# williamleif/GraphSAGE

Hardware: NVIDIA H100
Metric: seed_nodes_per_sec (higher is better)
Workload: dtype f32

## Files before the change

graphsage_b200/_lib.py:

```python
import ctypes
import os

import torch

_HERE = os.path.dirname(os.path.abspath(__file__))
LIB_PATH = os.path.join(_HERE, "csrc", "libgraphsage_b200.so")

ABI_VERSION = 2
GS_F32, GS_BF16 = 0, 1
ACT_NONE, ACT_RELU = 0, 1
COMBINE_ADD, COMBINE_CONCAT = 0, 1
MATH_FP32_SIMT, MATH_TF32X3, MATH_TF32, MATH_BF16 = 0, 1, 2, 3
MAX_SEGMENTS = 4

c_i32, c_i64, c_u64, c_vp = ctypes.c_int32, ctypes.c_int64, ctypes.c_uint64, ctypes.c_void_p


class Segment(ctypes.Structure):
    _fields_ = [("self_ids", c_vp), ("neigh_ids", c_vp), ("self_row0", c_i64), ("neigh_row0", c_i64),
                ("n", c_i64), ("k", c_i32), ("_pad", c_i32), ("out_row0", c_i64)]


MAX_SHARDS = 16


class ShardedTable(ctypes.Structure):
    _fields_ = [("base", c_vp * MAX_SHARDS), ("row_start", c_i64 * (MAX_SHARDS + 1)), ("n_shards", c_i32),
                ("my_shard", c_i32), ("n_global_rows", c_i64), ("zero_row", c_i64), ("remap", c_vp)]


class GemmPart(ctypes.Structure):
    _fields_ = [("A", c_vp), ("lda", c_i64), ("K", c_i32), ("B", c_vp), ("ldb", c_i64), ("N", c_i32)]


MAX_EMBED_LISTS = 8
MAX_UNIQUE_SAMPLED = 1024
UNIQUE_DRAW_BUDGET = 1 << 20


class EmbedGradList(ctypes.Structure):
    _fields_ = [("ids", c_vp), ("grad", c_vp), ("ldg", c_i64), ("n", c_i64), ("group", c_i32), ("scale", ctypes.c_float)]


class DropoutSite(ctypes.Structure):
    _fields_ = [("seed", c_u64), ("call", ctypes.c_uint32), ("rate", ctypes.c_float), ("call_dev", c_vp)]


_SIGNATURES = {
    "gs_version": (c_i32, []),
    "gs_last_error_string": (ctypes.c_char_p, []),
    "gs_set_tuning": (c_i32, [ctypes.c_char_p, c_i32]),
    "gs_sample_padded": (c_i32, [c_vp, c_i64, c_i32, c_vp, c_i64, c_i32, c_vp, c_u64, c_u64, c_vp, c_vp, c_vp]),
    "gs_sample_padded_khop": (c_i32, [c_vp, c_i64, c_i32, c_vp, c_i64, ctypes.POINTER(c_i32), c_i32, c_u64, c_u64, c_vp,
                                      ctypes.POINTER(c_vp), c_vp]),
    "gs_build_padded_adj": (c_i32, [c_vp, c_vp, c_i64, c_i32, c_vp, c_u64, c_u64, c_vp, c_vp, c_vp]),
    "gs_sample_unigram": (c_i32, [c_vp, c_i64, c_i32, c_u64, c_u64, c_vp, c_vp, c_vp]),
    "gs_sample_unigram_unique": (c_i32, [c_vp, c_i64, c_i32, c_u64, c_u64, c_vp, c_vp, c_vp, c_vp]),
    "gs_sample_csr": (c_i32, [c_vp, c_vp, c_i64, c_vp, c_i64, c_i32, c_i32, c_u64, c_u64, c_vp, c_i32, c_vp, c_vp]),
    "gs_perm_prefix_host": (c_i32, [c_u64, c_u64, c_i32, c_i32, ctypes.POINTER(c_i32)]),
    "gs_gather_rows": (c_i32, [c_vp, c_i32, c_i64, c_i32, c_i64, c_vp, c_i64, c_vp, c_i64, c_vp]),
    "gs_gather_mean": (c_i32, [c_vp, c_i32, c_i64, c_i32, c_i64, ctypes.POINTER(Segment), c_i32, c_i32, c_vp, c_vp,
                               c_i64, c_vp]),
    "gs_gather_mean_sharded": (c_i32, [ctypes.POINTER(ShardedTable), c_i32, c_i32, c_i64, ctypes.POINTER(Segment), c_i32,
                                       c_i32, c_i32, c_vp, c_vp, c_vp, c_i64, c_vp]),
    "gs_halo_begin": (c_i32, [c_vp, c_i64, c_vp, c_vp]),
    "gs_halo_claim": (c_i32, [ctypes.POINTER(ShardedTable), c_vp, c_i64, c_vp, c_vp, c_vp, c_i64, c_vp]),
    "gs_halo_fetch": (c_i32, [ctypes.POINTER(ShardedTable), c_i32, c_i64, c_vp, c_vp, c_i64, c_vp, c_i64, c_vp]),
    "gs_halo_translate": (c_i32, [ctypes.POINTER(ShardedTable), c_vp, c_i64, c_vp, c_vp, c_vp]),
    "gs_translate_ids": (c_i32, [ctypes.POINTER(ShardedTable), c_vp, c_i64, c_vp, c_vp]),
    "gs_gather_rows_sharded": (c_i32, [ctypes.POINTER(ShardedTable), c_i32, c_i32, c_i64, c_vp, c_i64, c_vp, c_i64, c_vp]),
    "gs_shard_alloc": (c_i32, [c_i64, ctypes.POINTER(c_vp)]),
    "gs_shard_free": (c_i32, [c_vp]),
    "gs_ipc_export": (c_i32, [c_vp, ctypes.c_char_p]),
    "gs_ipc_import": (c_i32, [ctypes.c_char_p, ctypes.POINTER(c_vp)]),
    "gs_ipc_close": (c_i32, [c_vp]),
    "gs_gather_rows_f32": (c_i32, [c_vp, c_i32, c_i64, c_i32, c_i64, c_vp, c_i64, c_i64, c_vp, c_i64, c_vp]),
    "gs_cast_rows_bf16": (c_i32, [c_vp, c_i64, c_i32, c_i64, c_vp, c_i64, c_vp]),
    "gs_rmat_degrees": (c_i32, [c_i32, c_i64, ctypes.c_double, ctypes.c_double, ctypes.c_double, ctypes.c_double,
                                ctypes.c_double, c_u64, c_u64, c_u64, c_u64, c_vp, c_vp]),
    "gs_rmat_fill": (c_i32, [c_i32, c_i64, ctypes.c_double, ctypes.c_double, ctypes.c_double, ctypes.c_double, c_u64, c_u64,
                             c_u64, c_u64, c_vp, c_vp, c_vp, c_i64, c_i64, c_vp]),
    "gs_segment_max": (c_i32, [c_vp, c_i64, c_i32, c_i32, c_i64, c_vp, c_i64, c_vp]),
    "gs_sage_gemm_workspace_bytes": (c_i64, [c_i64, ctypes.POINTER(GemmPart), c_i32, c_i32]),
    "gs_sage_gemm": (c_i32, [c_i64, ctypes.POINTER(GemmPart), c_i32, c_i32, c_vp, c_i32, c_i32, c_vp, c_i64, c_vp,
                             c_vp]),
    "gs_sage_gemm_pack": (c_i32, [ctypes.POINTER(GemmPart), c_i32, c_i32, c_vp, c_vp]),
    "gs_sage_gemm_prepacked": (c_i32, [c_i64, ctypes.POINTER(GemmPart), c_i32, c_i32, c_vp, c_i32, c_i32, c_vp, c_i64,
                                       c_vp, c_vp]),
    "gs_gather_mean_img_bytes": (c_i64, [c_i64, c_i32, c_i32]),
    "gs_gather_mean_img": (c_i32, [c_vp, c_i64, ctypes.POINTER(ShardedTable), c_i32, c_vp, c_i32, c_i64, ctypes.POINTER(Segment),
                                   c_i32, c_i32, c_i32, c_vp, c_vp]),
    "gs_sage_gemm_img": (c_i32, [c_i64, ctypes.POINTER(GemmPart), c_i32, c_i32, c_vp, c_i32, c_vp, c_i64, c_vp, c_vp, c_i32,
                                 c_vp]),
    "gs_sage_layer_small": (c_i32, [c_vp, c_i64, c_i32, c_i64, ctypes.POINTER(Segment), c_i32, ctypes.POINTER(GemmPart),
                                    c_i32, c_i32, c_vp, c_i32, c_i32, c_vp, c_i64, c_vp, c_u64, c_vp]),
    "gs_maxpool_mlp_workspace_bytes": (c_i64, [c_i32, c_i32]),
    "gs_maxpool_mlp_pack": (c_i32, [c_vp, c_i64, c_i32, c_i32, c_vp, c_vp]),
    "gs_maxpool_mlp_fused": (c_i32, [c_vp, c_i64, c_i32, c_i64, c_vp, c_i64, c_i64, c_i32, c_vp, c_vp, c_i32, c_vp, c_i64,
                                     c_vp]),
    "gs_meanpool_mlp_fused": (c_i32, [c_vp, c_i64, c_i32, c_i64, c_vp, c_i64, c_i64, c_i32, c_vp, c_vp, c_i32, c_vp, c_i64,
                                      c_vp]),
    "gs_pipeline_step": (c_i32, [c_vp, c_vp, c_i64, ctypes.POINTER(c_vp), c_i32, c_vp, c_vp, c_i64, c_vp, c_vp, c_vp, c_vp,
                                 c_vp, c_vp]),
    "gs_l2_normalize_rows": (c_i32, [c_vp, c_i64, c_i32, c_i64, c_vp]),
    "gs_bump_counter": (c_i32, [c_vp, c_u64, c_vp]),
    "gs_embedding_grad_workspace_bytes": (c_i64, [ctypes.POINTER(EmbedGradList), c_i32, c_i64, c_i32]),
    "gs_embedding_grad": (c_i32, [ctypes.POINTER(EmbedGradList), c_i32, c_i64, c_i32, c_vp, c_i64, c_vp, c_i64, c_vp]),
    "gs_gather_mean_dropout": (c_i32, [c_vp, c_i64, c_i32, c_i64, ctypes.POINTER(Segment), c_i32, ctypes.POINTER(DropoutSite),
                                       ctypes.POINTER(DropoutSite), c_i32, c_vp, c_vp, c_i64, c_vp]),
    "gs_dropout_apply": (c_i32, [c_vp, c_i64, c_i64, c_i32, c_i32, ctypes.c_float, DropoutSite, c_i32, c_vp, c_i64, c_vp]),
    "gs_embedding_grad_dropout": (c_i32, [ctypes.POINTER(EmbedGradList), ctypes.POINTER(DropoutSite), c_i32, c_i64, c_i32, c_vp,
                                          c_i64, c_vp, c_i64, c_vp]),
    "gs_embedding_sgd": (c_i32, [ctypes.POINTER(EmbedGradList), c_i32, c_i64, c_i32, ctypes.c_float, c_vp, c_i64, c_vp, c_i64,
                                 c_vp]),
    "gs_skipgram_workspace_bytes": (c_i64, [c_i64, c_i32, c_i32]),
    "gs_skipgram_grad": (c_i32, [c_vp, c_i64, c_vp, c_i64, c_i64, c_i32, c_vp, c_vp, c_i64, c_vp, c_i32, c_vp, c_vp, c_vp, c_vp,
                                 c_i64, c_vp, c_vp, c_i64, c_vp, c_i64, c_vp]),
}

_lib = None


def lib():
    global _lib
    if _lib is None:
        if not os.path.exists(LIB_PATH):
            raise ImportError(
                "graphsage_b200: %s is missing - build it with `python -m graphsage_b200.build` "
                "(there is no CPU fallback)" % LIB_PATH)
        _lib = ctypes.CDLL(LIB_PATH)
        for name, (res, args) in _SIGNATURES.items():
            fn = getattr(_lib, name)
            fn.restype, fn.argtypes = res, args
        if _lib.gs_version() != ABI_VERSION:
            raise ImportError("graphsage_b200: %s has ABI version %d, this binding needs %d - rebuild it"
                              % (LIB_PATH, _lib.gs_version(), ABI_VERSION))
        for kv in os.environ.get("GS_TUNING", "").split(","):
            if "=" in kv:
                k, v = kv.split("=", 1)
                _lib.gs_set_tuning(k.strip().encode(), int(v))
    return _lib


def exported_symbols():
    return sorted(_SIGNATURES)


def check(rc):
    if rc != 0:
        msg = lib().gs_last_error_string().decode("utf-8", "replace")
        raise RuntimeError("libgraphsage_b200 error %d: %s" % (rc, msg))


def stream_ptr():
    return torch.cuda.current_stream().cuda_stream


def ptr(t):
    return 0 if t is None else t.data_ptr()


def require_cuda(*tensors):
    for t in tensors:
        if t is not None and not t.is_cuda:
            raise RuntimeError("graphsage_b200: tensor on %s - the hot path is CUDA-only (no CPU fallback)" % t.device)


def set_tuning(key, value):
    return lib().gs_set_tuning(key.encode(), int(value))


def perm_prefix_host(seed, counter, max_deg, k):
    buf = (c_i32 * max(k, 1))()
    check(lib().gs_perm_prefix_host(seed & (2**64 - 1), counter & (2**64 - 1), max_deg, k, buf))
    return list(buf[:k])
```

graphsage_b200/csrc/gather.cu:

```cuda
#include "common.cuh"

namespace gs {

struct SegTable {
  gs_segment s[GS_MAX_SEGMENTS];
  int32_t n_segments;
  int64_t total_rows;
};

__device__ __forceinline__ int find_segment(const SegTable& t, int64_t r, int64_t& local) {
  int si = 0;
  int64_t base = 0, end = 0;
#pragma unroll
  for (int q = 0; q < GS_MAX_SEGMENTS - 1; ++q) {
    if (q < t.n_segments - 1) {
      end += t.s[q].n;
      if (r >= end) {
        base = end;
        si = q + 1;
      }
    }
  }
  local = r - base;
  return si;
}

__device__ __forceinline__ int64_t clamp_row(int64_t id, int64_t n_rows) {
  return (id < 0 || id >= n_rows) ? n_rows - 1 : id;
}

__device__ __forceinline__ float4 mask_tail(float4 v, int col0, int F) {
  if (col0 + 1 >= F) v.y = 0.f;
  if (col0 + 2 >= F) v.z = 0.f;
  if (col0 + 3 >= F) v.w = 0.f;
  return v;
}

template <int kUnroll>
__global__ void __launch_bounds__(256) gather_mean_ldg_kernel(const float* __restrict__ src, int64_t n_src_rows, int F,
                                                              int64_t pitch, const __grid_constant__ SegTable tab, int include_self,
                                                              float* __restrict__ out_self,
                                                              float* __restrict__ out_mean, int64_t out_pitch) {
  const int ncol4 = (int)(out_pitch >> 2);
  for (int64_t r = blockIdx.x; r < tab.total_rows; r += gridDim.x) {
    int64_t i;
    const gs_segment& sg = tab.s[find_segment(tab, r, i)];
    const int k = sg.k;
    const int64_t orow = sg.out_row0 + i;
    const int64_t srow = clamp_row(sg.self_ids ? (int64_t)sg.self_ids[i] : sg.self_row0 + i, n_src_rows);
    for (int c = threadIdx.x; c < ncol4; c += blockDim.x) {
      const int col0 = c * 4;
      float4 acc = make_float4(0.f, 0.f, 0.f, 0.f);
      float4 sv = acc;
      if (col0 < F) {
        int j = 0;
        for (; j + kUnroll <= k; j += kUnroll) {
          float4 v[kUnroll];
#pragma unroll
          for (int u = 0; u < kUnroll; ++u) {
            int64_t nr = clamp_row(sg.neigh_ids ? (int64_t)sg.neigh_ids[i * k + j + u] : sg.neigh_row0 + i * k + j + u,
                                   n_src_rows);
            v[u] = ldg_nc_f4(reinterpret_cast<const float4*>(src + nr * pitch) + c);
          }
#pragma unroll
          for (int u = 0; u < kUnroll; ++u) {
            acc.x += v[u].x; acc.y += v[u].y; acc.z += v[u].z; acc.w += v[u].w;
          }
        }
        for (; j < k; ++j) {
          int64_t nr = clamp_row(sg.neigh_ids ? (int64_t)sg.neigh_ids[i * k + j] : sg.neigh_row0 + i * k + j, n_src_rows);
          float4 v = ldg_nc_f4(reinterpret_cast<const float4*>(src + nr * pitch) + c);
          acc.x += v.x; acc.y += v.y; acc.z += v.z; acc.w += v.w;
        }
        if (include_self || out_self) sv = ldg_nc_f4(reinterpret_cast<const float4*>(src + srow * pitch) + c);
        float div = (float)(k + (include_self ? 1 : 0));
        if (include_self) { acc.x += sv.x; acc.y += sv.y; acc.z += sv.z; acc.w += sv.w; }
        acc.x /= div; acc.y /= div; acc.z /= div; acc.w /= div;
        acc = mask_tail(acc, col0, F);
        sv = mask_tail(sv, col0, F);
      }
      reinterpret_cast<float4*>(out_mean + orow * out_pitch)[c] = acc;
      if (out_self) reinterpret_cast<float4*>(out_self + orow * out_pitch)[c] = sv;
    }
  }
}

struct DropTab {
  DropSite neigh[GS_MAX_SEGMENTS];
  DropSite self[GS_MAX_SEGMENTS];
};

template <bool kDrop>
__global__ void __launch_bounds__(256) gather_mean_scalar_kernel(const float* __restrict__ src, int64_t n_src_rows, int F,
                                                                 int64_t pitch, const __grid_constant__ SegTable tab, int include_self,
                                                                 float* __restrict__ out_self,
                                                                 float* __restrict__ out_mean, int64_t out_pitch,
                                                                 const __grid_constant__ DropTab drop) {
  __shared__ uint32_t drop_off[2 * GS_MAX_SEGMENTS];
  if constexpr (kDrop) {
    if (threadIdx.x < 2 * GS_MAX_SEGMENTS) {
      const int s = threadIdx.x % GS_MAX_SEGMENTS;
      drop_off[threadIdx.x] = drop_call_offset(threadIdx.x < GS_MAX_SEGMENTS ? drop.neigh[s] : drop.self[s]);
    }
    __syncthreads();
  }
  for (int64_t r = blockIdx.x; r < tab.total_rows; r += gridDim.x) {
    int64_t i;
    const int si = find_segment(tab, r, i);
    const gs_segment& sg = tab.s[si];
    const int k = sg.k;
    const int64_t orow = sg.out_row0 + i;
    const int64_t srow = clamp_row(sg.self_ids ? (int64_t)sg.self_ids[i] : sg.self_row0 + i, n_src_rows);
    DropSite nsite{}, ssite{};
    if constexpr (kDrop) {
      nsite = with_call_offset(drop.neigh[si], drop_off[si]);
      ssite = with_call_offset(drop.self[si], drop_off[GS_MAX_SEGMENTS + si]);
    }
    for (int c = threadIdx.x; c < (int)out_pitch; c += blockDim.x) {
      float acc = 0.f, sv = 0.f;
      if (c < F) {
        for (int j = 0; j < k; ++j) {
          int64_t nr = clamp_row(sg.neigh_ids ? (int64_t)sg.neigh_ids[i * k + j] : sg.neigh_row0 + i * k + j, n_src_rows);
          if constexpr (kDrop) acc += drop_col(nsite, i * k + j, c, src[nr * pitch + c]);
          else acc += src[nr * pitch + c];
        }
        sv = src[srow * pitch + c];
        if constexpr (kDrop) sv = drop_col(ssite, i, c, sv);
        if (include_self) acc += sv;
        acc /= (float)(k + (include_self ? 1 : 0));
      }
      out_mean[orow * out_pitch + c] = acc;
      if (out_self) out_self[orow * out_pitch + c] = sv;
    }
  }
}

__global__ void __launch_bounds__(192) gather_mean_tma_kernel(const float* __restrict__ src, int64_t n_src_rows, int F,
                                                              int64_t pitch, const __grid_constant__ SegTable tab, int include_self,
                                                              float* __restrict__ out_self,
                                                              float* __restrict__ out_mean, int64_t out_pitch,
                                                              int row_bytes) {
  extern __shared__ __align__(128) unsigned char smem[];
  __shared__ __align__(8) uint64_t bar;
  if (threadIdx.x == 0) {
    mbar_init(&bar, 1);
    fence_mbar_init();
  }
  __syncthreads();
  const int ncol4 = (int)(out_pitch >> 2);
  const int row_f4 = row_bytes >> 4;
  uint32_t phase = 0;
  for (int64_t r = blockIdx.x; r < tab.total_rows; r += gridDim.x) {
    int64_t i;
    const gs_segment& sg = tab.s[find_segment(tab, r, i)];
    const int k = sg.k;
    const int64_t orow = sg.out_row0 + i;
    if (threadIdx.x < 32) {
      if (threadIdx.x == 0) mbar_expect_tx(&bar, (uint32_t)((k + 1) * row_bytes));
      __syncwarp();
      for (int j = threadIdx.x; j <= k; j += 32) {
        int64_t id;
        if (j < k) id = sg.neigh_ids ? (int64_t)sg.neigh_ids[i * k + j] : sg.neigh_row0 + i * k + j;
        else id = sg.self_ids ? (int64_t)sg.self_ids[i] : sg.self_row0 + i;
        id = clamp_row(id, n_src_rows);
        bulk_g2s(smem + (size_t)j * row_bytes, src + id * pitch, (uint32_t)row_bytes, &bar);
      }
    }
    mbar_wait(&bar, phase);
    phase ^= 1u;
    const float4* rows = reinterpret_cast<const float4*>(smem);
    for (int c = threadIdx.x; c < ncol4; c += blockDim.x) {
      const int col0 = c * 4;
      float4 acc = make_float4(0.f, 0.f, 0.f, 0.f);
      float4 sv = acc;
      if (col0 < F) {
#pragma unroll 5
        for (int j = 0; j < k; ++j) {
          float4 v = rows[j * row_f4 + c];
          acc.x += v.x; acc.y += v.y; acc.z += v.z; acc.w += v.w;
        }
        sv = rows[k * row_f4 + c];
        float div = (float)(k + (include_self ? 1 : 0));
        if (include_self) { acc.x += sv.x; acc.y += sv.y; acc.z += sv.z; acc.w += sv.w; }
        acc.x /= div; acc.y /= div; acc.z /= div; acc.w /= div;
        acc = mask_tail(acc, col0, F);
        sv = mask_tail(sv, col0, F);
      }
      reinterpret_cast<float4*>(out_mean + orow * out_pitch)[c] = acc;
      if (out_self) reinterpret_cast<float4*>(out_self + orow * out_pitch)[c] = sv;
    }
    __syncthreads();
  }
}

struct DenseRows {
  const float* src;
  int64_t n_rows, pitch;
  __device__ __forceinline__ const float* row(int64_t id) const { return src + clamp_row(id, n_rows) * pitch; }
};

struct ShardTab {
  const float* base[GS_MAX_SHARDS];
  int64_t row_start[GS_MAX_SHARDS + 1];
  int32_t n_shards, my_shard;
  int64_t n_global_rows;
  int64_t zero_row;
  const int32_t* remap;
};

struct ShardRows {
  ShardTab t;
  int64_t pitch;
  int32_t locators;
  const float* staging;
  __device__ __forceinline__ const float* row(int64_t id) const {
    const float* mine = t.base[t.my_shard];
    if (locators) {
      if (id >= 0) return mine + id * pitch;
      if (locators == 2) return staging + (-id - 1) * pitch;
      id = -id - 1;
    } else if (id < 0 || id >= t.n_global_rows - 1) {
      return mine + t.zero_row * pitch;
    } else if (t.remap) {
      const int32_t s = __ldg(t.remap + id);
      if (s >= 0) return mine + (int64_t)s * pitch;
    } else if (id >= t.row_start[t.my_shard] && id < t.row_start[t.my_shard + 1]) {
      return mine + (id - t.row_start[t.my_shard]) * pitch;
    }
    int o = 0;
#pragma unroll
    for (int q = 1; q < GS_MAX_SHARDS; ++q)
      if (q < t.n_shards && id >= t.row_start[q]) o = q;
    return t.base[o] + (id - t.row_start[o]) * pitch;
  }
};

constexpr int kGroupRows = 13;

struct GatherImg {
  unsigned char* base;
  int32_t kblocks, n_mtiles;
  int32_t want_self;
};

__device__ __forceinline__ void gather_img_store(const GatherImg& im, int part, int64_t orow, int c, float4 v) {
  const int kb = c >> 3, chunk = c & 7;
  const int64_t mt = orow >> 7;
  const int r = (int)(orow & 127);
  unsigned char* dst = im.base + ((((int64_t)part * im.n_mtiles + mt) * im.kblocks + kb) * 2) * 16384 +
                       (uint32_t)(r * 128 + ((chunk ^ (r & 7)) << 4));
  uint4 hi, lo;
  hi.x = __float_as_uint(v.x) & 0xFFFFE000u; hi.y = __float_as_uint(v.y) & 0xFFFFE000u;
  hi.z = __float_as_uint(v.z) & 0xFFFFE000u; hi.w = __float_as_uint(v.w) & 0xFFFFE000u;
  lo.x = __float_as_uint(v.x - __uint_as_float(hi.x)) & 0xFFFFE000u; lo.y = __float_as_uint(v.y - __uint_as_float(hi.y)) & 0xFFFFE000u;
  lo.z = __float_as_uint(v.z - __uint_as_float(hi.z)) & 0xFFFFE000u; lo.w = __float_as_uint(v.w - __uint_as_float(hi.w)) & 0xFFFFE000u;
  *reinterpret_cast<uint4*>(dst) = hi;
  *reinterpret_cast<uint4*>(dst + 16384) = lo;
}

template <class Rows, bool kDrop>
__global__ void __launch_bounds__(192) gather_mean_tma2_kernel(const __grid_constant__ Rows rows_of, int F,
                                                               const __grid_constant__ SegTable tab,
                                                               int include_self, float* __restrict__ out_self,
                                                               float* __restrict__ out_mean, int64_t out_pitch,
                                                               int row_bytes, const __grid_constant__ GatherImg img,
                                                               const __grid_constant__ DropTab drop) {
  extern __shared__ __align__(128) unsigned char smem[];
  __shared__ __align__(8) uint64_t bar[2];
  __shared__ uint32_t drop_off[2 * GS_MAX_SEGMENTS];
  if (threadIdx.x == 0) {
    mbar_init(&bar[0], 1);
    mbar_init(&bar[1], 1);
    fence_mbar_init();
  }
  if constexpr (kDrop) {
    if (threadIdx.x < 2 * GS_MAX_SEGMENTS) {
      const int s = threadIdx.x % GS_MAX_SEGMENTS;
      drop_off[threadIdx.x] = drop_call_offset(threadIdx.x < GS_MAX_SEGMENTS ? drop.neigh[s] : drop.self[s]);
    }
  }
  __syncthreads();
  const int ncol4 = (int)(out_pitch >> 2);
  const int row_f4 = row_bytes >> 4;
  const size_t buf_bytes = (size_t)kGroupRows * row_bytes;

  int64_t r_issue = blockIdx.x;
  int g_issue = 0;
  auto issue = [&](int buf) -> bool {
    if (r_issue >= tab.total_rows) return false;
    int64_t i;
    const gs_segment& sg = tab.s[find_segment(tab, r_issue, i)];
    const int k = sg.k;
    const int rows_total = k + 1;
    const int first = g_issue * kGroupRows;
    const int cnt = min(kGroupRows, rows_total - first);
    if (threadIdx.x < 32) {
      if (threadIdx.x == 0) mbar_expect_tx(&bar[buf], (uint32_t)(cnt * row_bytes));
      __syncwarp();
      for (int j = threadIdx.x; j < cnt; j += 32) {
        const int jj = first + j;
        int64_t id;
        if (jj < k) id = sg.neigh_ids ? (int64_t)sg.neigh_ids[i * k + jj] : sg.neigh_row0 + i * k + jj;
        else id = sg.self_ids ? (int64_t)sg.self_ids[i] : sg.self_row0 + i;
        bulk_g2s(smem + buf * buf_bytes + (size_t)j * row_bytes, rows_of.row(id), (uint32_t)row_bytes, &bar[buf]);
      }
    }
    if (first + cnt >= rows_total) { r_issue += gridDim.x; g_issue = 0; } else { ++g_issue; }
    return true;
  };

  uint32_t phase[2] = {0u, 0u};
  int buf = 0;
  bool have = issue(0);
  int64_t r = blockIdx.x;
  int g = 0;
  float4 acc[2];
  acc[0] = acc[1] = make_float4(0.f, 0.f, 0.f, 0.f);
  while (have) {
    const bool have_next = issue(buf ^ 1);
    int64_t i;
    const int si = find_segment(tab, r, i);
    const gs_segment& sg = tab.s[si];
    const int k = sg.k;
    const int rows_total = k + 1;
    const int first = g * kGroupRows;
    const int cnt = min(kGroupRows, rows_total - first);
    const bool last = first + cnt >= rows_total;
    mbar_wait(&bar[buf], phase[buf]);
    phase[buf] ^= 1u;
    const float4* rows = reinterpret_cast<const float4*>(smem + buf * buf_bytes);
    const int nn = last ? cnt - 1 : cnt;
    DropSite nsite{};
    if constexpr (kDrop) nsite = with_call_offset(drop.neigh[si], drop_off[si]);
#pragma unroll
    for (int q = 0; q < 2; ++q) {
      const int c = threadIdx.x + q * blockDim.x;
      if (c < ncol4 && c * 4 < F) {
        float4 a = acc[q];
        for (int j = 0; j < nn; ++j) {
          float4 v = rows[j * row_f4 + c];
          if constexpr (kDrop) v = drop4(nsite, i * k + first + j, (uint32_t)c, v);
          a.x += v.x; a.y += v.y; a.z += v.z; a.w += v.w;
        }
        acc[q] = a;
      }
    }
    if (last) {
      const int64_t orow = sg.out_row0 + i;
      const int ncol_img = img.base ? img.kblocks * 8 : 0;
#pragma unroll
      for (int q = 0; q < 2; ++q) {
        const int c = threadIdx.x + q * blockDim.x;
        if (c < ncol4 || c < ncol_img) {
          float4 a = make_float4(0.f, 0.f, 0.f, 0.f), sv = a;
          if (c < ncol4 && c * 4 < F) {
            a = acc[q];
            sv = rows[(cnt - 1) * row_f4 + c];
            if constexpr (kDrop) sv = drop4(with_call_offset(drop.self[si], drop_off[GS_MAX_SEGMENTS + si]), i, (uint32_t)c, sv);
            const float div = (float)(k + (include_self ? 1 : 0));
            if (include_self) { a.x += sv.x; a.y += sv.y; a.z += sv.z; a.w += sv.w; }
            a.x /= div; a.y /= div; a.z /= div; a.w /= div;
            a = mask_tail(a, c * 4, F);
            sv = mask_tail(sv, c * 4, F);
          }
          if (c < ncol4) {
            if (out_mean) reinterpret_cast<float4*>(out_mean + orow * out_pitch)[c] = a;
            if (out_self) reinterpret_cast<float4*>(out_self + orow * out_pitch)[c] = sv;
          }
          if (c < ncol_img) {
            if (img.want_self) gather_img_store(img, 0, orow, c, sv);
            gather_img_store(img, img.want_self ? 1 : 0, orow, c, a);
          }
          if (c < ncol4) acc[q] = make_float4(0.f, 0.f, 0.f, 0.f);
        }
      }
      r += gridDim.x;
      g = 0;
    } else {
      ++g;
    }
    __syncthreads();
    buf ^= 1;
    have = have_next;
  }
}

__global__ void __launch_bounds__(192) gather_mean_bf16_tma2_kernel(const uint16_t* __restrict__ src, int64_t n_src_rows, int F,
                                                                    int64_t pitch, const __grid_constant__ SegTable tab,
                                                                    int include_self, float* __restrict__ out_self,
                                                                    float* __restrict__ out_mean, int64_t out_pitch,
                                                                    int row_bytes) {
  extern __shared__ __align__(128) unsigned char smem[];
  __shared__ __align__(8) uint64_t bar[2];
  if (threadIdx.x == 0) {
    mbar_init(&bar[0], 1);
    mbar_init(&bar[1], 1);
    fence_mbar_init();
  }
  __syncthreads();
  const int ncol8 = (int)(out_pitch >> 3);
  const int row_u4 = row_bytes >> 4;
  const size_t buf_bytes = (size_t)kGroupRows * row_bytes;
  int64_t r_issue = blockIdx.x;
  int g_issue = 0;
  auto issue = [&](int buf) -> bool {
    if (r_issue >= tab.total_rows) return false;
    int64_t i;
    const gs_segment& sg = tab.s[find_segment(tab, r_issue, i)];
    const int k = sg.k;
    const int rows_total = k + 1;
    const int first = g_issue * kGroupRows;
    const int cnt = min(kGroupRows, rows_total - first);
    if (threadIdx.x < 32) {
      if (threadIdx.x == 0) mbar_expect_tx(&bar[buf], (uint32_t)(cnt * row_bytes));
      __syncwarp();
      for (int j = threadIdx.x; j < cnt; j += 32) {
        const int jj = first + j;
        int64_t id;
        if (jj < k) id = sg.neigh_ids ? (int64_t)sg.neigh_ids[i * k + jj] : sg.neigh_row0 + i * k + jj;
        else id = sg.self_ids ? (int64_t)sg.self_ids[i] : sg.self_row0 + i;
        id = clamp_row(id, n_src_rows);
        bulk_g2s(smem + buf * buf_bytes + (size_t)j * row_bytes, src + id * pitch, (uint32_t)row_bytes, &bar[buf]);
      }
    }
    if (first + cnt >= rows_total) { r_issue += gridDim.x; g_issue = 0; } else { ++g_issue; }
    return true;
  };
  auto widen = [](uint4 u, float (&v)[8]) {
    const uint32_t w[4] = {u.x, u.y, u.z, u.w};
#pragma unroll
    for (int e = 0; e < 4; ++e) {
      v[2 * e] = __uint_as_float(w[e] << 16);
      v[2 * e + 1] = __uint_as_float(w[e] & 0xffff0000u);
    }
  };
  uint32_t phase[2] = {0u, 0u};
  int buf = 0;
  bool have = issue(0);
  int64_t r = blockIdx.x;
  int g = 0;
  float acc[8];
#pragma unroll
  for (int e = 0; e < 8; ++e) acc[e] = 0.f;
  const int c = threadIdx.x;
  while (have) {
    const bool have_next = issue(buf ^ 1);
    int64_t i;
    const gs_segment& sg = tab.s[find_segment(tab, r, i)];
    const int k = sg.k;
    const int rows_total = k + 1;
    const int first = g * kGroupRows;
    const int cnt = min(kGroupRows, rows_total - first);
    const bool last = first + cnt >= rows_total;
    mbar_wait(&bar[buf], phase[buf]);
    phase[buf] ^= 1u;
    const uint4* rows = reinterpret_cast<const uint4*>(smem + buf * buf_bytes);
    const int nn = last ? cnt - 1 : cnt;
    if (c < ncol8 && c * 8 < F) {
      for (int j = 0; j < nn; ++j) {
        float v[8];
        widen(rows[j * row_u4 + c], v);
#pragma unroll
        for (int e = 0; e < 8; ++e) acc[e] += v[e];
      }
    }
    if (last) {
      const int64_t orow = sg.out_row0 + i;
      if (c < ncol8) {
        float a[8], sv[8];
#pragma unroll
        for (int e = 0; e < 8; ++e) { a[e] = 0.f; sv[e] = 0.f; }
        if (c * 8 < F) {
          widen(rows[(cnt - 1) * row_u4 + c], sv);
          const float div = (float)(k + (include_self ? 1 : 0));
#pragma unroll
          for (int e = 0; e < 8; ++e) {
            float t = acc[e];
            if (include_self) t += sv[e];
            a[e] = (c * 8 + e < F) ? t / div : 0.f;
            if (c * 8 + e >= F) sv[e] = 0.f;
          }
        }
        float4* om = reinterpret_cast<float4*>(out_mean + orow * out_pitch) + 2 * c;
        om[0] = make_float4(a[0], a[1], a[2], a[3]);
        om[1] = make_float4(a[4], a[5], a[6], a[7]);
        if (out_self) {
          float4* os = reinterpret_cast<float4*>(out_self + orow * out_pitch) + 2 * c;
          os[0] = make_float4(sv[0], sv[1], sv[2], sv[3]);
          os[1] = make_float4(sv[4], sv[5], sv[6], sv[7]);
        }
#pragma unroll
        for (int e = 0; e < 8; ++e) acc[e] = 0.f;
      }
      r += gridDim.x;
      g = 0;
    } else {
      ++g;
    }
    __syncthreads();
    buf ^= 1;
    have = have_next;
  }
}

__global__ void __launch_bounds__(32) gather_rows_tma_kernel(const unsigned char* __restrict__ src, int64_t n_rows,
                                                             int64_t pitch_bytes, const int32_t* __restrict__ ids,
                                                             int64_t n, unsigned char* __restrict__ out,
                                                             int64_t out_pitch_bytes, int row_bytes) {
  extern __shared__ __align__(128) unsigned char smem[];
  __shared__ __align__(8) uint64_t bar;
  const int lane = threadIdx.x;
  if (lane == 0) {
    mbar_init(&bar, 1);
    fence_mbar_init();
  }
  __syncwarp();
  uint32_t phase = 0;
  for (int64_t base = (int64_t)blockIdx.x * 32; base < n; base += (int64_t)gridDim.x * 32) {
    int cnt = (int)((n - base) < 32 ? (n - base) : 32);
    if (lane == 0) mbar_expect_tx(&bar, (uint32_t)(cnt * row_bytes));
    __syncwarp();
    if (lane < cnt) {
      int64_t id = clamp_row(ids[base + lane], n_rows);
      bulk_g2s(smem + (size_t)lane * row_bytes, src + id * pitch_bytes, (uint32_t)row_bytes, &bar);
    }
    mbar_wait(&bar, phase);
    phase ^= 1u;
    if (lane < cnt) bulk_s2g(out + (base + lane) * out_pitch_bytes, smem + (size_t)lane * row_bytes, (uint32_t)row_bytes);
    bulk_commit();
    bulk_wait_read<0>();
    __syncwarp();
  }
  bulk_wait<0>();
}

template <typename T>
__global__ void __launch_bounds__(256) gather_rows_simple_kernel(const T* __restrict__ src, int64_t n_rows, int F,
                                                                 int64_t pitch, const int32_t* __restrict__ ids,
                                                                 int64_t n, T* __restrict__ out, int64_t out_pitch) {
  const int lane = threadIdx.x & 31;
  const int64_t warp = ((int64_t)blockIdx.x * blockDim.x + threadIdx.x) >> 5;
  const int64_t nwarps = ((int64_t)gridDim.x * blockDim.x) >> 5;
  for (int64_t i = warp; i < n; i += nwarps) {
    int64_t id = clamp_row(ids[i], n_rows);
    for (int c = lane; c < F; c += 32) out[i * out_pitch + c] = src[id * pitch + c];
  }
}

template <typename T>
__global__ void __launch_bounds__(256) gather_rows_to_f32_kernel(const T* __restrict__ src, int64_t n_rows, int F,
                                                                 int64_t pitch, const int32_t* __restrict__ ids, int64_t row0,
                                                                 int64_t n, float* __restrict__ out, int64_t out_pitch) {
  const int lane = threadIdx.x & 31;
  const int64_t warp = ((int64_t)blockIdx.x * blockDim.x + threadIdx.x) >> 5;
  const int64_t nwarps = ((int64_t)gridDim.x * blockDim.x) >> 5;
  for (int64_t i = warp; i < n; i += nwarps) {
    const int64_t id = clamp_row(ids ? (int64_t)ids[i] : row0 + i, n_rows);
    for (int c = lane; c < (int)out_pitch; c += 32) {
      float v = 0.f;
      if (c < F) {
        if constexpr (sizeof(T) == 2) v = __uint_as_float(((uint32_t)src[id * pitch + c]) << 16);
        else v = src[id * pitch + c];
      }
      out[i * out_pitch + c] = v;
    }
  }
}

__global__ void __launch_bounds__(256) gather_rows_bf16_to_f32_vec_kernel(const uint16_t* __restrict__ src, int64_t n_rows, int F,
                                                                          int64_t pitch, const int32_t* __restrict__ ids,
                                                                          int64_t row0, int64_t n, float* __restrict__ out,
                                                                          int64_t out_pitch) {
  const int lane = threadIdx.x & 31;
  const int64_t warp = ((int64_t)blockIdx.x * blockDim.x + threadIdx.x) >> 5;
  const int64_t nwarps = ((int64_t)gridDim.x * blockDim.x) >> 5;
  const int chunks = (int)(out_pitch >> 3);
  for (int64_t i = warp; i < n; i += nwarps) {
    const int64_t id = clamp_row(ids ? (int64_t)ids[i] : row0 + i, n_rows);
    const uint4* rp = reinterpret_cast<const uint4*>(src + id * pitch);
    float4* op = reinterpret_cast<float4*>(out + i * out_pitch);
    for (int c = lane; c < chunks; c += 32) {
      uint4 u = make_uint4(0u, 0u, 0u, 0u);
      if (c * 8 < F) u = __ldg(rp + c);
      const uint32_t w[4] = {u.x, u.y, u.z, u.w};
      float v[8];
#pragma unroll
      for (int e = 0; e < 4; ++e) {
        v[2 * e] = (c * 8 + 2 * e < F) ? __uint_as_float(w[e] << 16) : 0.f;
        v[2 * e + 1] = (c * 8 + 2 * e + 1 < F) ? __uint_as_float(w[e] & 0xffff0000u) : 0.f;
      }
      op[2 * c] = make_float4(v[0], v[1], v[2], v[3]);
      op[2 * c + 1] = make_float4(v[4], v[5], v[6], v[7]);
    }
  }
}

__device__ __forceinline__ uint32_t f32_to_bf16_rne(float x) {
  const uint32_t u = __float_as_uint(x);
  if ((u & 0x7fffffffu) > 0x7f800000u) return (u >> 16) | 0x40u;
  return (u + 0x7fffu + ((u >> 16) & 1u)) >> 16;
}

__global__ void __launch_bounds__(256) cast_rows_bf16_kernel(const float* __restrict__ x, int64_t n, int F, int64_t ldx,
                                                             uint16_t* __restrict__ out, int64_t out_pitch) {
  const int chunks = (int)(out_pitch >> 3);
  const int64_t total = n * chunks;
  for (int64_t q = (int64_t)blockIdx.x * blockDim.x + threadIdx.x; q < total; q += (int64_t)gridDim.x * blockDim.x) {
    const int64_t i = q / chunks;
    const int c = (int)(q - i * chunks) * 8;
    const float* xp = x + i * ldx + c;
    uint32_t h[8];
#pragma unroll
    for (int e = 0; e < 8; ++e) h[e] = (c + e < F) ? f32_to_bf16_rne(xp[e]) : 0u;
    uint4 o;
    o.x = h[0] | (h[1] << 16); o.y = h[2] | (h[3] << 16); o.z = h[4] | (h[5] << 16); o.w = h[6] | (h[7] << 16);
    *reinterpret_cast<uint4*>(out + i * out_pitch + c) = o;
  }
}

__global__ void __launch_bounds__(256) cast_rows_bf16_scalar_kernel(const float* __restrict__ x, int64_t n, int F, int64_t ldx,
                                                                    uint16_t* __restrict__ out, int64_t out_pitch) {
  const int64_t total = n * out_pitch;
  for (int64_t q = (int64_t)blockIdx.x * blockDim.x + threadIdx.x; q < total; q += (int64_t)gridDim.x * blockDim.x) {
    const int64_t i = q / out_pitch;
    const int c = (int)(q - i * out_pitch);
    out[q] = c < F ? (uint16_t)f32_to_bf16_rne(x[i * ldx + c]) : (uint16_t)0;
  }
}

__global__ void __launch_bounds__(256) dropout_apply_kernel(const float* x, int64_t ldx, int64_t rows, int F, int group,
                                                            float scale, DropSite site, int accumulate, float* out,
                                                            int64_t ldo) {
  const int nc4 = (F + 3) >> 2;
  const int64_t total = rows * nc4;
  site.call += drop_call_offset(site);
  for (int64_t q = (int64_t)blockIdx.x * blockDim.x + threadIdx.x; q < total; q += (int64_t)gridDim.x * blockDim.x) {
    const int64_t r = q / nc4;
    const int c4 = (int)(q - r * nc4);
    const u32x4 w = drop_words(site, r, (uint32_t)c4);
    const float* xr = x + (r / group) * ldx;
    float* orow = out + r * ldo;
#pragma unroll
    for (int e = 0; e < 4; ++e) {
      const int c = c4 * 4 + e;
      if (c < F) {
        const float v = pick(w, e) >= site.threshold ? (xr[c] * scale) / site.keep : 0.f;
        orow[c] = accumulate ? orow[c] + v : v;
      }
    }
  }
}

__global__ void bump_counter_kernel(unsigned long long* counter, unsigned long long inc) { *counter += inc; }

__global__ void __launch_bounds__(256) segment_max_kernel(const float* __restrict__ x, int64_t n, int k, int C,
                                                          int64_t ldx, float* __restrict__ out, int64_t ldo) {
  for (int64_t i = blockIdx.x; i < n; i += gridDim.x) {
    for (int c = threadIdx.x; c < C; c += blockDim.x) {
      float m = x[(i * k) * ldx + c];
      for (int j = 1; j < k; ++j) m = fmaxf(m, x[(i * k + j) * ldx + c]);
      out[i * ldo + c] = m;
    }
  }
}

__global__ void __launch_bounds__(256) l2_normalize_kernel(float* __restrict__ x, int64_t n, int C, int64_t ldx) {
  const int lane = threadIdx.x & 31;
  const int64_t warp = ((int64_t)blockIdx.x * blockDim.x + threadIdx.x) >> 5;
  const int64_t nwarps = ((int64_t)gridDim.x * blockDim.x) >> 5;
  for (int64_t i = warp; i < n; i += nwarps) {
    float ss = 0.f;
    for (int c = lane; c < C; c += 32) {
      float v = x[i * ldx + c];
      ss += v * v;
    }
#pragma unroll
    for (int o = 16; o > 0; o >>= 1) ss += __shfl_xor_sync(0xffffffffu, ss, o);
    float inv = 1.0f / sqrtf(fmaxf(ss, 1e-12f));
    for (int c = lane; c < C; c += 32) x[i * ldx + c] *= inv;
  }
}

__global__ void __launch_bounds__(256) translate_ids_kernel(const int32_t* __restrict__ remap, int64_t n_global_rows,
                                                            int32_t zero_row, const int32_t* __restrict__ ids, int64_t n,
                                                            int32_t* __restrict__ out) {
  for (int64_t i = (int64_t)blockIdx.x * blockDim.x + threadIdx.x; i < n; i += (int64_t)gridDim.x * blockDim.x) {
    const int32_t id = ids[i];
    int32_t loc;
    if (id < 0 || id >= n_global_rows - 1) loc = zero_row;
    else {
      loc = __ldg(remap + id);
      if (loc < 0) loc = -id - 1;
    }
    out[i] = loc;
  }
}

__device__ __forceinline__ bool halo_is_local(const ShardTab& t, int32_t id, int32_t& loc) {
  if (id < 0 || id >= t.n_global_rows - 1) { loc = (int32_t)t.zero_row; return true; }
  if (t.remap) {
    loc = __ldg(t.remap + id);
    return loc >= 0;
  }
  if (id >= t.row_start[t.my_shard] && id < t.row_start[t.my_shard + 1]) { loc = (int32_t)(id - t.row_start[t.my_shard]); return true; }
  return false;
}

__global__ void __launch_bounds__(256) halo_claim_kernel(const __grid_constant__ ShardTab t, const int32_t* __restrict__ ids,
                                                         int64_t n, int32_t* __restrict__ claim, int32_t* __restrict__ count,
                                                         int32_t* __restrict__ stage_ids, int64_t capacity) {
  for (int64_t i = (int64_t)blockIdx.x * blockDim.x + threadIdx.x; i < n; i += (int64_t)gridDim.x * blockDim.x) {
    const int32_t id = ids[i];
    int32_t loc;
    if (halo_is_local(t, id, loc)) continue;
    if (atomicCAS(claim + id, -1, -2) == -1) {
      const int32_t idx = atomicAdd(count, 1);
      if (idx < capacity) stage_ids[idx] = id;
      claim[id] = idx;
    }
  }
}

__global__ void __launch_bounds__(256) halo_translate_kernel(const __grid_constant__ ShardTab t, const int32_t* __restrict__ ids,
                                                             int64_t n, const int32_t* __restrict__ claim,
                                                             int32_t* __restrict__ out) {
  for (int64_t i = (int64_t)blockIdx.x * blockDim.x + threadIdx.x; i < n; i += (int64_t)gridDim.x * blockDim.x) {
    const int32_t id = ids[i];
    int32_t loc;
    if (!halo_is_local(t, id, loc)) loc = -claim[id] - 1;
    out[i] = loc;
  }
}

constexpr int kHaloLoads = 5;
__global__ void __launch_bounds__(256) halo_fetch_kernel(const __grid_constant__ ShardRows sr, int row_f4,
                                                         const int32_t* __restrict__ stage_ids, const int32_t* __restrict__ count,
                                                         int64_t capacity, float* __restrict__ staging, int64_t staging_pitch) {
  const int lane = threadIdx.x & 31;
  const int64_t warp = ((int64_t)blockIdx.x * blockDim.x + threadIdx.x) >> 5;
  const int64_t nwarps = ((int64_t)gridDim.x * blockDim.x) >> 5;
  int64_t n = *count;
  if (n > capacity) n = capacity;
  for (int64_t i = warp; i < n; i += nwarps) {
    const float4* src = reinterpret_cast<const float4*>(sr.row(stage_ids[i]));
    float4* dst = reinterpret_cast<float4*>(staging + i * staging_pitch);
    for (int c0 = lane; c0 < row_f4; c0 += 32 * kHaloLoads) {
      float4 v[kHaloLoads];
#pragma unroll
      for (int u = 0; u < kHaloLoads; ++u)
        if (c0 + 32 * u < row_f4) v[u] = ldg_nc_f4(src + c0 + 32 * u);
#pragma unroll
      for (int u = 0; u < kHaloLoads; ++u)
        if (c0 + 32 * u < row_f4) dst[c0 + 32 * u] = v[u];
    }
  }
}

template <int kUnroll>
__global__ void __launch_bounds__(256) gather_mean_sharded_kernel(const __grid_constant__ ShardRows st, int F,
                                                                  const __grid_constant__ SegTable tab, int include_self,
                                                                  float* __restrict__ out_self,
                                                                  float* __restrict__ out_mean, int64_t out_pitch) {
  const int ncol4 = (int)(out_pitch >> 2);
  for (int64_t r = blockIdx.x; r < tab.total_rows; r += gridDim.x) {
    int64_t i;
    const gs_segment& sg = tab.s[find_segment(tab, r, i)];
    const int k = sg.k;
    const int64_t orow = sg.out_row0 + i;
    const float* srow = st.row(sg.self_ids ? (int64_t)sg.self_ids[i] : sg.self_row0 + i);
    for (int c = threadIdx.x; c < ncol4; c += blockDim.x) {
      const int col0 = c * 4;
      float4 acc = make_float4(0.f, 0.f, 0.f, 0.f);
      float4 sv = acc;
      if (col0 < F) {
        int j = 0;
        for (; j + kUnroll <= k; j += kUnroll) {
          float4 v[kUnroll];
#pragma unroll
          for (int u = 0; u < kUnroll; ++u) {
            const float* p = st.row(sg.neigh_ids ? (int64_t)sg.neigh_ids[i * k + j + u] : sg.neigh_row0 + i * k + j + u);
            v[u] = ldg_nc_f4(reinterpret_cast<const float4*>(p) + c);
          }
#pragma unroll
          for (int u = 0; u < kUnroll; ++u) {
            acc.x += v[u].x; acc.y += v[u].y; acc.z += v[u].z; acc.w += v[u].w;
          }
        }
        for (; j < k; ++j) {
          const float* p = st.row(sg.neigh_ids ? (int64_t)sg.neigh_ids[i * k + j] : sg.neigh_row0 + i * k + j);
          float4 v = ldg_nc_f4(reinterpret_cast<const float4*>(p) + c);
          acc.x += v.x; acc.y += v.y; acc.z += v.z; acc.w += v.w;
        }
        if (include_self || out_self) sv = ldg_nc_f4(reinterpret_cast<const float4*>(srow) + c);
        float div = (float)(k + (include_self ? 1 : 0));
        if (include_self) { acc.x += sv.x; acc.y += sv.y; acc.z += sv.z; acc.w += sv.w; }
        acc.x /= div; acc.y /= div; acc.z /= div; acc.w /= div;
        acc = mask_tail(acc, col0, F);
        sv = mask_tail(sv, col0, F);
      }
      reinterpret_cast<float4*>(out_mean + orow * out_pitch)[c] = acc;
      if (out_self) reinterpret_cast<float4*>(out_self + orow * out_pitch)[c] = sv;
    }
  }
}

__global__ void __launch_bounds__(256) gather_rows_sharded_kernel(const __grid_constant__ ShardRows st, int F,
                                                                  const int32_t* __restrict__ ids, int64_t n,
                                                                  float* __restrict__ out, int64_t out_pitch) {
  const int lane = threadIdx.x & 31;
  const int64_t warp = ((int64_t)blockIdx.x * blockDim.x + threadIdx.x) >> 5;
  const int64_t nwarps = ((int64_t)gridDim.x * blockDim.x) >> 5;
  const int ncol4 = (int)(out_pitch >> 2);
  for (int64_t i = warp; i < n; i += nwarps) {
    const float* p = st.row(ids[i]);
    for (int c = lane; c < ncol4; c += 32) {
      float4 v = make_float4(0.f, 0.f, 0.f, 0.f);
      if (c * 4 < F) v = mask_tail(ldg_nc_f4(reinterpret_cast<const float4*>(p) + c), c * 4, F);
      reinterpret_cast<float4*>(out + i * out_pitch)[c] = v;
    }
  }
}

static inline bool aligned16(const void* p) { return (reinterpret_cast<uintptr_t>(p) & 15u) == 0; }

}


namespace gs {
template <class Rows, bool kDrop = false>
static int32_t launch_gather_tma2(const Rows& rows_of, int F, const SegTable& tab, int include_self, float* out_self, float* out_mean,
                                  int64_t out_pitch, const GatherImg& img, cudaStream_t st, const DropTab* drop = nullptr) {
  const int32_t rc_attr = ensure_dyn_smem((const void*)gather_mean_tma2_kernel<Rows, kDrop>, 200 * 1024);
  if (rc_attr != GS_OK) return rc_attr;
  const int ncol4 = (int)(out_pitch / 4);
  const int row_bytes = ((F + 3) / 4) * 16;
  const size_t smem2 = (size_t)2 * kGroupRows * row_bytes;
  int threads = ((ncol4 + 31) / 32) * 32;
  if (threads > 160) threads = 160;
  if (threads < 32) threads = 32;
  int per_sm = (int)((224 * 1024) / (smem2 + 1024));
  if (per_sm < 1) per_sm = 1;
  int lim = tuning("gather_ctas_per_sm", 8);
  if (per_sm > lim) per_sm = lim;
  int64_t blocks = tab.total_rows;
  int64_t cap = (int64_t)sm_count() * per_sm;
  if (blocks > cap) blocks = cap;
  DropTab no_drop;
  memset(&no_drop, 0, sizeof(no_drop));
  gather_mean_tma2_kernel<Rows, kDrop><<<(unsigned)blocks, threads, smem2, st>>>(rows_of, F, tab, include_self, out_self,
                                                                                 out_mean, out_pitch, row_bytes, img,
                                                                                 drop ? *drop : no_drop);
  return launch_check("gather_mean_tma2_kernel");
}
}

extern "C" {

int32_t gs_gather_rows(const void* feats, int32_t dtype, int64_t n_rows, int32_t F, int64_t pitch, const int32_t* ids,
                       int64_t n, void* out, int64_t out_pitch, void* stream) {
  GS_REQUIRE(n >= 0 && F >= 0, "gs_gather_rows: negative size");
  if (n == 0 || F == 0) return GS_OK;
  GS_REQUIRE(feats && ids && out, "gs_gather_rows: NULL pointer");
  GS_REQUIRE(dtype == GS_F32 || dtype == GS_BF16, "gs_gather_rows: dtype %d", dtype);
  GS_REQUIRE(n_rows > 0 && pitch >= F && out_pitch >= F, "gs_gather_rows: pitch < F");
  const int es = dtype == GS_F32 ? 4 : 2;
  cudaStream_t st = (cudaStream_t)stream;
  const int row_bytes = ((F * es + 15) / 16) * 16;
  const bool tma_ok = gs::aligned16(feats) && gs::aligned16(out) && (pitch * es) % 16 == 0 && (out_pitch * es) % 16 == 0 &&
                      row_bytes <= pitch * es && row_bytes <= out_pitch * es && row_bytes * 32 <= 200 * 1024;
  if (tma_ok && gs::tuning("gather_variant", 2) != 0) {
    size_t smem = (size_t)row_bytes * 32;
    {
      const int32_t rc_attr = gs::ensure_dyn_smem((const void*)gs::gather_rows_tma_kernel, 200 * 1024);
      if (rc_attr != GS_OK) return rc_attr;
    }
    int per_sm = (int)((220 * 1024) / (smem + 1024));
    if (per_sm < 1) per_sm = 1;
    if (per_sm > 16) per_sm = 16;
    int64_t blocks = (n + 31) / 32;
    int64_t cap = (int64_t)gs::sm_count() * per_sm;
    if (blocks > cap) blocks = cap;
    gs::gather_rows_tma_kernel<<<(unsigned)blocks, 32, smem, st>>>((const unsigned char*)feats, n_rows, pitch * es, ids, n,
                                                                   (unsigned char*)out, out_pitch * es, row_bytes);
    return gs::launch_check("gather_rows_tma_kernel");
  }
  int64_t blocks = (n + 7) / 8;
  int64_t cap = (int64_t)gs::sm_count() * 8;
  if (blocks > cap) blocks = cap;
  if (dtype == GS_F32)
    gs::gather_rows_simple_kernel<float><<<(unsigned)blocks, 256, 0, st>>>((const float*)feats, n_rows, F, pitch, ids, n,
                                                                           (float*)out, out_pitch);
  else
    gs::gather_rows_simple_kernel<uint16_t><<<(unsigned)blocks, 256, 0, st>>>((const uint16_t*)feats, n_rows, F, pitch, ids,
                                                                              n, (uint16_t*)out, out_pitch);
  return gs::launch_check("gather_rows_simple_kernel");
}

int32_t gs_gather_mean(const void* src, int32_t dtype, int64_t n_src_rows, int32_t F, int64_t pitch,
                       const gs_segment* segments_host, int32_t n_segments, int32_t include_self, void* out_self,
                       void* out_mean, int64_t out_pitch, void* stream) {
  GS_REQUIRE(dtype == GS_F32 || dtype == GS_BF16, "gs_gather_mean: dtype %d (GS_F32 or GS_BF16)", dtype);
  GS_REQUIRE(n_segments >= 0 && n_segments <= GS_MAX_SEGMENTS, "gs_gather_mean: n_segments=%d (max %d)", n_segments,
             GS_MAX_SEGMENTS);
  GS_REQUIRE(segments_host || n_segments == 0, "gs_gather_mean: segments_host is NULL");
  gs::SegTable tab;
  memset(&tab, 0, sizeof(tab));
  tab.n_segments = n_segments;
  int kmax = 0;
  for (int s = 0; s < n_segments; ++s) {
    tab.s[s] = segments_host[s];
    GS_REQUIRE(tab.s[s].n >= 0 && tab.s[s].k >= 1, "gs_gather_mean: segment %d has n=%lld k=%d", s, (long long)tab.s[s].n,
               tab.s[s].k);
    tab.total_rows += tab.s[s].n;
    if (tab.s[s].k > kmax) kmax = tab.s[s].k;
  }
  if (tab.total_rows == 0) return GS_OK;
  GS_REQUIRE(src && out_mean, "gs_gather_mean: NULL pointer");
  GS_REQUIRE(F > 0 && pitch >= F && out_pitch >= F && n_src_rows > 0, "gs_gather_mean: bad F/pitch");
  cudaStream_t st = (cudaStream_t)stream;
  if (dtype == GS_BF16) {
    const int64_t f8 = ((int64_t)F + 7) / 8 * 8;
    if (!(gs::aligned16(src) && gs::aligned16(out_mean) && (!out_self || gs::aligned16(out_self)) && pitch % 8 == 0 &&
          out_pitch % 8 == 0 && f8 <= pitch && f8 <= out_pitch && f8 / 8 <= 192)) {
      gs::set_error("gs_gather_mean(GS_BF16): needs 16-byte aligned rows (pitch %% 8 == 0), out_pitch %% 8 == 0 and F <= 1536");
      return GS_ERR_UNSUPPORTED;
    }
    const int32_t rc_attr = gs::ensure_dyn_smem((const void*)gs::gather_mean_bf16_tma2_kernel, 200 * 1024);
    if (rc_attr != GS_OK) return rc_attr;
    const int row_bytes = (int)(f8 * 2);
    const size_t smem2 = (size_t)2 * gs::kGroupRows * row_bytes;
    const int ncol8 = (int)(out_pitch / 8);
    int threads = ((ncol8 + 31) / 32) * 32;
    if (threads < 32) threads = 32;
    GS_REQUIRE(threads <= 192, "gs_gather_mean(GS_BF16): out_pitch too wide");
    int per_sm = (int)((224 * 1024) / (smem2 + 1024));
    if (per_sm < 1) per_sm = 1;
    int lim = gs::tuning("gather_ctas_per_sm", 8);
    if (per_sm > lim) per_sm = lim;
    int64_t blocks = tab.total_rows;
    int64_t cap = (int64_t)gs::sm_count() * per_sm;
    if (blocks > cap) blocks = cap;
    gs::gather_mean_bf16_tma2_kernel<<<(unsigned)blocks, threads, smem2, st>>>((const uint16_t*)src, n_src_rows, F, pitch, tab,
                                                                              include_self, (float*)out_self, (float*)out_mean,
                                                                              out_pitch, row_bytes);
    return gs::launch_check("gather_mean_bf16_tma2_kernel");
  }
  const float* fsrc = (const float*)src;
  const bool vec_ok = gs::aligned16(src) && gs::aligned16(out_mean) && (!out_self || gs::aligned16(out_self)) &&
                      pitch % 4 == 0 && out_pitch % 4 == 0 && ((F + 3) / 4) * 4 <= pitch;
  if (!vec_ok) {
    int64_t blocks = tab.total_rows;
    int64_t cap = (int64_t)gs::sm_count() * 8;
    if (blocks > cap) blocks = cap;
    gs::DropTab no_drop;
    memset(&no_drop, 0, sizeof(no_drop));
    gs::gather_mean_scalar_kernel<false><<<(unsigned)blocks, 256, 0, st>>>(fsrc, n_src_rows, F, pitch, tab, include_self,
                                                                           (float*)out_self, (float*)out_mean, out_pitch,
                                                                           no_drop);
    return gs::launch_check("gather_mean_scalar_kernel");
  }
  const int ncol4 = (int)(out_pitch / 4);
  const int row_bytes = ((F + 3) / 4) * 16;
  const size_t smem = (size_t)row_bytes * (kmax + 1);
  const int variant = gs::tuning("gather_variant", 2);
  if (variant == 2 && ncol4 <= 2 * 160) {
    const gs::DenseRows rows_of{fsrc, n_src_rows, pitch};
    gs::GatherImg img;
    memset(&img, 0, sizeof(img));
    return gs::launch_gather_tma2(rows_of, F, tab, include_self, (float*)out_self, (float*)out_mean, out_pitch, img, st);
  }
  if (variant >= 1 && smem <= 200 * 1024) {
    {
      const int32_t rc_attr = gs::ensure_dyn_smem((const void*)gs::gather_mean_tma_kernel, 200 * 1024);
      if (rc_attr != GS_OK) return rc_attr;
    }
    int threads = ((ncol4 + 31) / 32) * 32;
    if (threads > 192) threads = 192;
    if (threads < 32) threads = 32;
    int per_sm = (int)((224 * 1024) / (smem + 1024));
    if (per_sm < 1) per_sm = 1;
    int lim = gs::tuning("gather_ctas_per_sm", 8);
    if (per_sm > lim) per_sm = lim;
    int64_t blocks = tab.total_rows;
    int64_t cap = (int64_t)gs::sm_count() * per_sm;
    if (blocks > cap) blocks = cap;
    gs::gather_mean_tma_kernel<<<(unsigned)blocks, threads, smem, st>>>(fsrc, n_src_rows, F, pitch, tab, include_self,
                                                                        (float*)out_self, (float*)out_mean, out_pitch,
                                                                        row_bytes);
    return gs::launch_check("gather_mean_tma_kernel");
  }
  int threads = ((ncol4 + 31) / 32) * 32;
  if (threads > 256) threads = 256;
  int64_t blocks = tab.total_rows;
  int64_t cap = (int64_t)gs::sm_count() * gs::tuning("gather_ctas_per_sm", 8);
  if (blocks > cap) blocks = cap;
  gs::gather_mean_ldg_kernel<5><<<(unsigned)blocks, threads, 0, st>>>(fsrc, n_src_rows, F, pitch, tab, include_self,
                                                                      (float*)out_self, (float*)out_mean, out_pitch);
  return gs::launch_check("gather_mean_ldg_kernel");
}

int32_t gs_gather_rows_f32(const void* feats, int32_t dtype, int64_t n_rows, int32_t F, int64_t pitch, const int32_t* ids,
                           int64_t row0, int64_t n, float* out, int64_t out_pitch, void* stream) {
  GS_REQUIRE(n >= 0 && F >= 0, "gs_gather_rows_f32: negative size");
  if (n == 0 || out_pitch == 0) return GS_OK;
  GS_REQUIRE(feats && out, "gs_gather_rows_f32: NULL pointer");
  GS_REQUIRE(dtype == GS_F32 || dtype == GS_BF16, "gs_gather_rows_f32: dtype %d", dtype);
  GS_REQUIRE(n_rows > 0 && pitch >= F && out_pitch >= F, "gs_gather_rows_f32: pitch < F");
  int64_t blocks = (n + 7) / 8;
  int64_t cap = (int64_t)gs::sm_count() * 8;
  if (blocks > cap) blocks = cap;
  if (dtype == GS_F32)
    gs::gather_rows_to_f32_kernel<float><<<(unsigned)blocks, 256, 0, (cudaStream_t)stream>>>(
        (const float*)feats, n_rows, F, pitch, ids, row0, n, out, out_pitch);
  else if (pitch % 8 == 0 && out_pitch % 8 == 0 && gs::aligned16(feats) && gs::aligned16(out) && out_pitch <= pitch)
    gs::gather_rows_bf16_to_f32_vec_kernel<<<(unsigned)blocks, 256, 0, (cudaStream_t)stream>>>(
        (const uint16_t*)feats, n_rows, F, pitch, ids, row0, n, out, out_pitch);
  else
    gs::gather_rows_to_f32_kernel<uint16_t><<<(unsigned)blocks, 256, 0, (cudaStream_t)stream>>>(
        (const uint16_t*)feats, n_rows, F, pitch, ids, row0, n, out, out_pitch);
  return gs::launch_check("gather_rows_to_f32_kernel");
}

int32_t gs_cast_rows_bf16(const float* x, int64_t n, int32_t F, int64_t ldx, void* out_bf16, int64_t out_pitch,
                          void* stream) {
  GS_REQUIRE(n >= 0 && F >= 0 && ldx >= F && out_pitch >= F, "gs_cast_rows_bf16: bad sizes");
  if (n == 0 || out_pitch == 0) return GS_OK;
  GS_REQUIRE(x && out_bf16, "gs_cast_rows_bf16: NULL pointer");
  const bool vec = out_pitch % 8 == 0 && gs::aligned16(out_bf16) && ldx >= ((F + 7) / 8) * 8;
  int64_t blocks = ((vec ? n * (out_pitch / 8) : n * out_pitch) + 255) / 256;
  int64_t cap = (int64_t)gs::sm_count() * 8;
  if (blocks > cap) blocks = cap;
  if (vec)
    gs::cast_rows_bf16_kernel<<<(unsigned)blocks, 256, 0, (cudaStream_t)stream>>>(x, n, F, ldx, (uint16_t*)out_bf16, out_pitch);
  else
    gs::cast_rows_bf16_scalar_kernel<<<(unsigned)blocks, 256, 0, (cudaStream_t)stream>>>(x, n, F, ldx, (uint16_t*)out_bf16,
                                                                                         out_pitch);
  return gs::launch_check("cast_rows_bf16_kernel");
}

int32_t gs_bump_counter(uint64_t* counter_dev, uint64_t inc, void* stream) {
  GS_REQUIRE(counter_dev != nullptr, "gs_bump_counter: NULL counter");
  gs::bump_counter_kernel<<<1, 1, 0, (cudaStream_t)stream>>>((unsigned long long*)counter_dev, (unsigned long long)inc);
  return gs::launch_check("bump_counter_kernel");
}

int32_t gs_segment_max(const float* x, int64_t n, int32_t k, int32_t C, int64_t ldx, float* out, int64_t ldo,
                       void* stream) {
  GS_REQUIRE(n >= 0 && k >= 1 && C >= 0, "gs_segment_max: bad sizes");
  if (n == 0 || C == 0) return GS_OK;
  GS_REQUIRE(x && out, "gs_segment_max: NULL pointer");
  int64_t blocks = n;
  int64_t cap = (int64_t)gs::sm_count() * 8;
  if (blocks > cap) blocks = cap;
  gs::segment_max_kernel<<<(unsigned)blocks, 256, 0, (cudaStream_t)stream>>>(x, n, k, C, ldx, out, ldo);
  return gs::launch_check("segment_max_kernel");
}

static int32_t check_site(const gs_dropout_site& s, const char* who) {
  GS_REQUIRE(s.rate >= 0.f && s.rate < 1.f, "%s: dropout rate %g outside [0, 1)", who, (double)s.rate);
  return GS_OK;
}

int32_t gs_gather_mean_dropout(const float* src, int64_t n_src_rows, int32_t F, int64_t pitch, const gs_segment* segments_host,
                               int32_t n_segments, const gs_dropout_site* neigh_sites_host,
                               const gs_dropout_site* self_sites_host, int32_t include_self, float* out_self,
                               float* out_mean, int64_t out_pitch, void* stream) {
  GS_REQUIRE(n_segments >= 0 && n_segments <= GS_MAX_SEGMENTS, "gs_gather_mean_dropout: n_segments=%d (max %d)", n_segments,
             GS_MAX_SEGMENTS);
  GS_REQUIRE((segments_host && neigh_sites_host && self_sites_host) || n_segments == 0,
             "gs_gather_mean_dropout: segments / sites are NULL");
  gs::SegTable tab;
  memset(&tab, 0, sizeof(tab));
  gs::DropTab drop;
  memset(&drop, 0, sizeof(drop));
  tab.n_segments = n_segments;
  for (int s = 0; s < n_segments; ++s) {
    tab.s[s] = segments_host[s];
    GS_REQUIRE(tab.s[s].n >= 0 && tab.s[s].k >= 1, "gs_gather_mean_dropout: segment %d has n=%lld k=%d", s,
               (long long)tab.s[s].n, tab.s[s].k);
    int32_t rc = check_site(neigh_sites_host[s], "gs_gather_mean_dropout");
    if (rc == GS_OK) rc = check_site(self_sites_host[s], "gs_gather_mean_dropout");
    if (rc != GS_OK) return rc;
    drop.neigh[s] = gs::make_drop_site(neigh_sites_host[s]);
    drop.self[s] = gs::make_drop_site(self_sites_host[s]);
    tab.total_rows += tab.s[s].n;
  }
  if (tab.total_rows == 0) return GS_OK;
  GS_REQUIRE(src && out_mean, "gs_gather_mean_dropout: NULL pointer");
  GS_REQUIRE(F > 0 && pitch >= F && out_pitch >= F && n_src_rows > 0, "gs_gather_mean_dropout: bad F/pitch");
  cudaStream_t st = (cudaStream_t)stream;
  const int ncol4 = (int)(out_pitch / 4);
  const bool vec_ok = gs::aligned16(src) && gs::aligned16(out_mean) && (!out_self || gs::aligned16(out_self)) &&
                      pitch % 4 == 0 && out_pitch % 4 == 0 && ((F + 3) / 4) * 4 <= pitch;
  if (vec_ok && ncol4 <= 2 * 160) {
    const gs::DenseRows rows_of{src, n_src_rows, pitch};
    gs::GatherImg img;
    memset(&img, 0, sizeof(img));
    return gs::launch_gather_tma2<gs::DenseRows, true>(rows_of, F, tab, include_self, out_self, out_mean, out_pitch, img, st,
                                                       &drop);
  }
  int64_t blocks = tab.total_rows;
  int64_t cap = (int64_t)gs::sm_count() * 8;
  if (blocks > cap) blocks = cap;
  gs::gather_mean_scalar_kernel<true><<<(unsigned)blocks, 256, 0, st>>>(src, n_src_rows, F, pitch, tab, include_self, out_self,
                                                                        out_mean, out_pitch, drop);
  return gs::launch_check("gather_mean_scalar_kernel<drop>");
}

int32_t gs_dropout_apply(const float* x, int64_t ldx, int64_t rows, int32_t F, int32_t group, float scale,
                         gs_dropout_site site, int32_t accumulate, float* out, int64_t ldo, void* stream) {
  int32_t rc = check_site(site, "gs_dropout_apply");
  if (rc != GS_OK) return rc;
  GS_REQUIRE(rows >= 0 && F >= 0 && group >= 1, "gs_dropout_apply: bad sizes (rows=%lld F=%d group=%d)", (long long)rows, F,
             group);
  if (rows == 0 || F == 0) return GS_OK;
  GS_REQUIRE(x && out, "gs_dropout_apply: NULL pointer");
  GS_REQUIRE(ldx >= F && ldo >= F, "gs_dropout_apply: row stride < F");
  GS_REQUIRE(x != out || (group == 1 && ldx == ldo), "gs_dropout_apply: in place needs group == 1 and ldo == ldx");
  const int64_t total = rows * ((F + 3) / 4);
  int64_t blocks = (total + 255) / 256;
  int64_t cap = (int64_t)gs::sm_count() * 16;
  if (blocks > cap) blocks = cap;
  gs::dropout_apply_kernel<<<(unsigned)blocks, 256, 0, (cudaStream_t)stream>>>(x, ldx, rows, F, group, scale,
                                                                                gs::make_drop_site(site), accumulate, out, ldo);
  return gs::launch_check("dropout_apply_kernel");
}

int32_t gs_l2_normalize_rows(float* x, int64_t n, int32_t C, int64_t ldx, void* stream) {
  GS_REQUIRE(n >= 0 && C >= 0, "gs_l2_normalize_rows: bad sizes");
  if (n == 0 || C == 0) return GS_OK;
  GS_REQUIRE(x, "gs_l2_normalize_rows: NULL pointer");
  int64_t blocks = (n + 7) / 8;
  int64_t cap = (int64_t)gs::sm_count() * 8;
  if (blocks > cap) blocks = cap;
  gs::l2_normalize_kernel<<<(unsigned)blocks, 256, 0, (cudaStream_t)stream>>>(x, n, C, ldx);
  return gs::launch_check("l2_normalize_kernel");
}

}

static int32_t fill_shard_tab(const gs_sharded_table* t, gs::ShardRows& sr, int64_t pitch, const char* who) {
  GS_REQUIRE(t != nullptr, "%s: table is NULL", who);
  GS_REQUIRE(t->n_shards >= 1 && t->n_shards <= GS_MAX_SHARDS, "%s: n_shards=%d (max %d)", who, t->n_shards, GS_MAX_SHARDS);
  GS_REQUIRE(t->my_shard >= 0 && t->my_shard < t->n_shards, "%s: my_shard=%d", who, t->my_shard);
  GS_REQUIRE(t->n_global_rows > 0 && t->row_start[0] == 0 && t->row_start[t->n_shards] == t->n_global_rows - 1,
             "%s: row_start must run from 0 to n_global_rows - 1", who);
  for (int i = 0; i < t->n_shards; ++i)
    GS_REQUIRE(t->row_start[i] <= t->row_start[i + 1], "%s: row_start must be non-decreasing (shard %d)", who, i);
  GS_REQUIRE(t->zero_row >= 0, "%s: zero_row < 0", who);
  GS_REQUIRE(pitch % 4 == 0, "%s: pitch must be a multiple of 4 floats", who);
  memset(&sr, 0, sizeof(sr));
  gs::ShardTab& st = sr.t;
  for (int i = 0; i < t->n_shards; ++i) {
    GS_REQUIRE(t->base[i] != nullptr && gs::aligned16(t->base[i]), "%s: shard %d pointer NULL or not 16-byte aligned", who, i);
    st.base[i] = (const float*)t->base[i];
  }
  for (int i = 0; i <= t->n_shards; ++i) st.row_start[i] = t->row_start[i];
  for (int i = t->n_shards + 1; i <= GS_MAX_SHARDS; ++i) st.row_start[i] = t->row_start[t->n_shards];
  st.n_shards = t->n_shards;
  st.my_shard = t->my_shard;
  st.n_global_rows = t->n_global_rows;
  st.zero_row = t->zero_row;
  st.remap = t->remap;
  sr.pitch = pitch;
  return GS_OK;
}

extern "C" {

int32_t gs_translate_ids(const gs_sharded_table* table_host, const int32_t* ids, int64_t n, int32_t* out, void* stream) {
  GS_REQUIRE(table_host && table_host->remap, "gs_translate_ids: the table has no remap (no replicas)");
  GS_REQUIRE(n >= 0, "gs_translate_ids: n < 0");
  if (n == 0) return GS_OK;
  GS_REQUIRE(ids && out, "gs_translate_ids: NULL pointer");
  GS_REQUIRE(table_host->zero_row >= 0 && table_host->zero_row < 0x7fffffffLL, "gs_translate_ids: zero_row out of range");
  int64_t blocks = (n + 255) / 256;
  int64_t cap = (int64_t)gs::sm_count() * 8;
  if (blocks > cap) blocks = cap;
  gs::translate_ids_kernel<<<(unsigned)blocks, 256, 0, (cudaStream_t)stream>>>(table_host->remap, table_host->n_global_rows,
                                                                                (int32_t)table_host->zero_row, ids, n, out);
  return gs::launch_check("translate_ids_kernel");
}

int64_t gs_gather_mean_img_bytes(int64_t rows, int32_t F, int32_t want_self) {
  if (rows < 0 || F < 1) return -1;
  const int64_t n_mtiles = (rows + 127) / 128, kblocks = (F + 31) / 32;
  return (want_self ? 2 : 1) * n_mtiles * kblocks * 2 * 16384;
}

int32_t gs_gather_mean_img(const void* src, int64_t n_src_rows, const gs_sharded_table* table_host, int32_t ids_are_locators,
                           const void* staging, int32_t F, int64_t pitch, const gs_segment* segments_host, int32_t n_segments,
                           int32_t include_self, int32_t want_self, void* images, void* stream) {
  GS_REQUIRE((src != nullptr) != (table_host != nullptr), "gs_gather_mean_img: pass either a dense table or a sharded one");
  GS_REQUIRE(n_segments >= 0 && n_segments <= GS_MAX_SEGMENTS && (segments_host || n_segments == 0),
             "gs_gather_mean_img: bad segments");
  gs::SegTable tab;
  memset(&tab, 0, sizeof(tab));
  tab.n_segments = n_segments;
  int64_t rows = 0;
  for (int s = 0; s < n_segments; ++s) {
    tab.s[s] = segments_host[s];
    GS_REQUIRE(tab.s[s].n >= 0 && tab.s[s].k >= 1, "gs_gather_mean_img: segment %d has n=%lld k=%d", s, (long long)tab.s[s].n,
               tab.s[s].k);
    tab.total_rows += tab.s[s].n;
    if (tab.s[s].out_row0 + tab.s[s].n > rows) rows = tab.s[s].out_row0 + tab.s[s].n;
  }
  if (tab.total_rows == 0) return GS_OK;
  GS_REQUIRE(images && (reinterpret_cast<uintptr_t>(images) & 1023u) == 0, "gs_gather_mean_img: images must be 1024-byte aligned");
  const int64_t out_pitch = ((int64_t)F + 7) / 8 * 8;
  const int ncol4 = (int)(out_pitch / 4);
  if (ncol4 > 2 * 160 || F < 1 || pitch % 4 != 0 || pitch < ((F + 3) / 4) * 4 || gs::tuning("gather_variant", 2) != 2) {
    gs::set_error("gs_gather_mean_img: needs F <= 1280, 16-byte row pitch and the bulk-copy gather (F=%d pitch=%lld)", F, (long long)pitch);
    return GS_ERR_UNSUPPORTED;
  }
  gs::GatherImg img;
  img.base = (unsigned char*)images;
  img.kblocks = (F + 31) / 32;
  img.n_mtiles = (int32_t)((rows + 127) / 128);
  img.want_self = want_self ? 1 : 0;
  if (src) {
    GS_REQUIRE(gs::aligned16(src) && n_src_rows > 0, "gs_gather_mean_img: table must be 16-byte aligned");
    const gs::DenseRows rows_of{(const float*)src, n_src_rows, pitch};
    return gs::launch_gather_tma2(rows_of, F, tab, include_self, nullptr, nullptr, out_pitch, img, (cudaStream_t)stream);
  }
  gs::ShardRows sr;
  int32_t rc = fill_shard_tab(table_host, sr, pitch, "gs_gather_mean_img");
  if (rc != GS_OK) return rc;
  GS_REQUIRE(ids_are_locators >= 0 && ids_are_locators <= 2 && (ids_are_locators != 2 || staging != nullptr),
             "gs_gather_mean_img: ids_are_locators = 2 needs the staging buffer");
  sr.locators = ids_are_locators;
  sr.staging = (const float*)staging;
  return gs::launch_gather_tma2(sr, F, tab, include_self, nullptr, nullptr, out_pitch, img, (cudaStream_t)stream);
}

int32_t gs_halo_begin(int32_t* claim, int64_t n_global_rows, int32_t* count, void* stream) {
  GS_REQUIRE(claim && count && n_global_rows > 0, "gs_halo_begin: bad arguments");
  GS_CUDA(cudaMemsetAsync(claim, 0xff, (size_t)n_global_rows * 4, (cudaStream_t)stream));
  GS_CUDA(cudaMemsetAsync(count, 0, 4, (cudaStream_t)stream));
  return GS_OK;
}

int32_t gs_halo_claim(const gs_sharded_table* table_host, const int32_t* ids, int64_t n, int32_t* claim, int32_t* count,
                      int32_t* stage_ids, int64_t capacity, void* stream) {
  gs::ShardRows sr;
  int32_t rc = fill_shard_tab(table_host, sr, 4, "gs_halo_claim");
  if (rc != GS_OK) return rc;
  GS_REQUIRE(n >= 0 && capacity >= 0, "gs_halo_claim: negative size");
  if (n == 0) return GS_OK;
  GS_REQUIRE(ids && claim && count && stage_ids, "gs_halo_claim: NULL pointer");
  int64_t blocks = (n + 255) / 256;
  int64_t cap = (int64_t)gs::sm_count() * 8;
  if (blocks > cap) blocks = cap;
  gs::halo_claim_kernel<<<(unsigned)blocks, 256, 0, (cudaStream_t)stream>>>(sr.t, ids, n, claim, count, stage_ids, capacity);
  return gs::launch_check("halo_claim_kernel");
}

int32_t gs_halo_translate(const gs_sharded_table* table_host, const int32_t* ids, int64_t n, const int32_t* claim, int32_t* out,
                          void* stream) {
  gs::ShardRows sr;
  int32_t rc = fill_shard_tab(table_host, sr, 4, "gs_halo_translate");
  if (rc != GS_OK) return rc;
  GS_REQUIRE(n >= 0, "gs_halo_translate: n < 0");
  if (n == 0) return GS_OK;
  GS_REQUIRE(ids && claim && out, "gs_halo_translate: NULL pointer");
  int64_t blocks = (n + 255) / 256;
  int64_t cap = (int64_t)gs::sm_count() * 8;
  if (blocks > cap) blocks = cap;
  gs::halo_translate_kernel<<<(unsigned)blocks, 256, 0, (cudaStream_t)stream>>>(sr.t, ids, n, claim, out);
  return gs::launch_check("halo_translate_kernel");
}

int32_t gs_halo_fetch(const gs_sharded_table* table_host, int32_t F, int64_t pitch, const int32_t* stage_ids,
                      const int32_t* count, int64_t capacity, float* staging, int64_t staging_pitch, void* stream) {
  gs::ShardRows sr;
  int32_t rc = fill_shard_tab(table_host, sr, pitch, "gs_halo_fetch");
  if (rc != GS_OK) return rc;
  if (capacity == 0) return GS_OK;
  GS_REQUIRE(stage_ids && count && staging && gs::aligned16(staging) && staging_pitch % 4 == 0 && F > 0 &&
                 pitch >= ((F + 3) / 4) * 4 && staging_pitch >= ((F + 3) / 4) * 4,
             "gs_halo_fetch: bad arguments");
  sr.locators = 0;
  sr.staging = nullptr;
  sr.t.remap = nullptr;
  const int blocks = gs::sm_count() * gs::tuning("halo_fetch_ctas_per_sm", 2);
  gs::halo_fetch_kernel<<<(unsigned)blocks, 256, 0, (cudaStream_t)stream>>>(sr, (F + 3) / 4, stage_ids, count, capacity, staging,
                                                                            staging_pitch);
  return gs::launch_check("halo_fetch_kernel");
}

int32_t gs_gather_mean_sharded(const gs_sharded_table* table_host, int32_t dtype, int32_t F, int64_t pitch,
                               const gs_segment* segments_host, int32_t n_segments, int32_t include_self,
                               int32_t ids_are_locators, const void* staging, void* out_self, void* out_mean,
                               int64_t out_pitch, void* stream) {
  GS_REQUIRE(dtype == GS_F32, "gs_gather_mean_sharded: only GS_F32 (dtype=%d)", dtype);
  GS_REQUIRE(n_segments >= 0 && n_segments <= GS_MAX_SEGMENTS && (segments_host || n_segments == 0),
             "gs_gather_mean_sharded: bad segments");
  gs::ShardRows sr;
  int32_t rc = fill_shard_tab(table_host, sr, pitch, "gs_gather_mean_sharded");
  if (rc != GS_OK) return rc;
  GS_REQUIRE(ids_are_locators >= 0 && ids_are_locators <= 2 && (ids_are_locators != 2 || staging != nullptr),
             "gs_gather_mean_sharded: ids_are_locators = 2 needs the staging buffer");
  sr.locators = ids_are_locators;
  sr.staging = (const float*)staging;
  gs::SegTable tab;
  memset(&tab, 0, sizeof(tab));
  tab.n_segments = n_segments;
  for (int s = 0; s < n_segments; ++s) {
    tab.s[s] = segments_host[s];
    GS_REQUIRE(tab.s[s].n >= 0 && tab.s[s].k >= 1, "gs_gather_mean_sharded: segment %d has n=%lld k=%d", s,
               (long long)tab.s[s].n, tab.s[s].k);
    tab.total_rows += tab.s[s].n;
  }
  if (tab.total_rows == 0) return GS_OK;
  GS_REQUIRE(out_mean && gs::aligned16(out_mean) && (!out_self || gs::aligned16(out_self)) && out_pitch % 4 == 0 &&
                 F > 0 && pitch >= ((F + 3) / 4) * 4 && out_pitch >= F,
             "gs_gather_mean_sharded: bad output / pitch");
  const int ncol4 = (int)(out_pitch / 4);
  if (gs::tuning("gather_variant", 2) != 0 && ncol4 <= 2 * 160) {
    gs::GatherImg img;
    memset(&img, 0, sizeof(img));
    return gs::launch_gather_tma2(sr, F, tab, include_self, (float*)out_self, (float*)out_mean, out_pitch, img,
                                  (cudaStream_t)stream);
  }
  int threads = ((ncol4 + 31) / 32) * 32;
  if (threads > 256) threads = 256;
  int64_t blocks = tab.total_rows;
  int64_t cap = (int64_t)gs::sm_count() * gs::tuning("gather_ctas_per_sm", 8);
  if (blocks > cap) blocks = cap;
  gs::gather_mean_sharded_kernel<5><<<(unsigned)blocks, threads, 0, (cudaStream_t)stream>>>(
      sr, F, tab, include_self, (float*)out_self, (float*)out_mean, out_pitch);
  return gs::launch_check("gather_mean_sharded_kernel");
}

int32_t gs_gather_rows_sharded(const gs_sharded_table* table_host, int32_t dtype, int32_t F, int64_t pitch,
                               const int32_t* ids, int64_t n, void* out, int64_t out_pitch, void* stream) {
  GS_REQUIRE(dtype == GS_F32, "gs_gather_rows_sharded: only GS_F32 (dtype=%d)", dtype);
  gs::ShardRows sr;
  int32_t rc = fill_shard_tab(table_host, sr, pitch, "gs_gather_rows_sharded");
  if (rc != GS_OK) return rc;
  if (n == 0) return GS_OK;
  GS_REQUIRE(ids && out && gs::aligned16(out) && out_pitch % 4 == 0 && F > 0 && pitch >= ((F + 3) / 4) * 4 && out_pitch >= F,
             "gs_gather_rows_sharded: bad arguments");
  int64_t blocks = (n + 7) / 8;
  int64_t cap = (int64_t)gs::sm_count() * 8;
  if (blocks > cap) blocks = cap;
  gs::gather_rows_sharded_kernel<<<(unsigned)blocks, 256, 0, (cudaStream_t)stream>>>(sr, F, ids, n, (float*)out, out_pitch);
  return gs::launch_check("gather_rows_sharded_kernel");
}

int32_t gs_shard_alloc(int64_t bytes, void** dev_ptr_out) {
  GS_REQUIRE(bytes > 0 && dev_ptr_out, "gs_shard_alloc: bad arguments");
  GS_CUDA(cudaMalloc(dev_ptr_out, (size_t)bytes));
  return GS_OK;
}

int32_t gs_shard_free(void* dev_ptr) {
  if (dev_ptr) GS_CUDA(cudaFree(dev_ptr));
  return GS_OK;
}

int32_t gs_ipc_export(const void* dev_ptr, uint8_t* handle64_out_host) {
  GS_REQUIRE(dev_ptr && handle64_out_host, "gs_ipc_export: NULL argument");
  static_assert(sizeof(cudaIpcMemHandle_t) == 64, "cudaIpcMemHandle_t is 64 bytes");
  cudaIpcMemHandle_t h;
  GS_CUDA(cudaIpcGetMemHandle(&h, const_cast<void*>(dev_ptr)));
  memcpy(handle64_out_host, &h, 64);
  return GS_OK;
}

int32_t gs_ipc_import(const uint8_t* handle64_host, void** dev_ptr_out) {
  GS_REQUIRE(handle64_host && dev_ptr_out, "gs_ipc_import: NULL argument");
  cudaIpcMemHandle_t h;
  memcpy(&h, handle64_host, 64);
  GS_CUDA(cudaIpcOpenMemHandle(dev_ptr_out, h, cudaIpcMemLazyEnablePeerAccess));
  return GS_OK;
}

int32_t gs_ipc_close(void* dev_ptr) {
  if (dev_ptr) GS_CUDA(cudaIpcCloseMemHandle(dev_ptr));
  return GS_OK;
}

}
```

graphsage_b200/ops.py:

```python
import torch

from . import _lib
from ._lib import (ACT_NONE, ACT_RELU, COMBINE_ADD, COMBINE_CONCAT, MATH_FP32_SIMT, MATH_TF32X3, MATH_TF32,
                   MATH_BF16, GemmPart, Segment, check, lib, ptr, require_cuda, stream_ptr)

_U64 = 2**64 - 1

PROBE = None
LAUNCHES = 0
STAGE_HOOK = None

CACHE_EPOCH = [0]
REPACK_ALWAYS = [False]


def _probe(name):
    if STAGE_HOOK is not None:
        STAGE_HOOK(name, "pre")
    if PROBE is None:
        return _PostHook(name) if STAGE_HOOK is not None else None
    e0, e1 = torch.cuda.Event(enable_timing=True), torch.cuda.Event(enable_timing=True)
    PROBE.setdefault(name, []).append((e0, e1))
    e0.record()
    return e1


class _PostHook(object):
    def __init__(self, name):
        self.name = name

    def record(self):
        if STAGE_HOOK is not None:
            STAGE_HOOK(self.name, "post")


def _launched(n=1, ev=None):
    global LAUNCHES
    LAUNCHES += n
    if ev is not None:
        ev.record()


def pad_cols(f):
    return (int(f) + 7) // 8 * 8


def _i32(t, name):
    if t.dtype != torch.int32:
        raise TypeError("%s must be int32 (got %s)" % (name, t.dtype))
    return t.contiguous()


def sample_padded(adj, ids, k, seed, counter, col_perm=None, counter_dev=None, out=None):
    require_cuda(adj, ids, col_perm, counter_dev)
    adj, ids = _i32(adj, "adj"), _i32(ids.reshape(-1), "ids")
    n = ids.numel()
    if out is None:
        out = torch.empty((n, k), dtype=torch.int32, device=adj.device)
    ev = _probe("sample_padded")
    check(lib().gs_sample_padded(ptr(adj), adj.shape[0], adj.shape[1], ptr(ids), n, k, ptr(col_perm), seed & _U64,
                                 counter & _U64, ptr(counter_dev), ptr(out), stream_ptr()))
    _launched(1 if n * k else 0, ev)
    return out


def sample_padded_khop(adj, seeds, fanouts, seed, counter, counter_dev=None):
    require_cuda(adj, seeds, counter_dev)
    adj, seeds = _i32(adj, "adj"), _i32(seeds.reshape(-1), "seeds")
    n = seeds.numel()
    outs, cnt = [], n
    for k in fanouts:
        cnt *= int(k)
        outs.append(torch.empty((cnt,), dtype=torch.int32, device=adj.device))
    fan = (_lib.c_i32 * len(fanouts))(*[int(k) for k in fanouts])
    optr = (_lib.c_vp * len(fanouts))(*[ptr(o) for o in outs])
    ev = _probe("sample_padded_khop")
    check(lib().gs_sample_padded_khop(ptr(adj), adj.shape[0], adj.shape[1], ptr(seeds), n, fan, len(fanouts),
                                      seed & _U64, counter & _U64, ptr(counter_dev), optr, stream_ptr()))
    _launched(1 if n else 0, ev)
    return outs


def build_padded_adj(indptr, indices, max_degree, seed=123, counter=0, skip=None):
    require_cuda(indptr, indices, skip)
    if indptr.dtype != torch.int64:
        raise TypeError("indptr must be int64")
    indices = _i32(indices, "indices")
    n = indptr.numel() - 1
    adj = torch.empty((n + 1, max_degree), dtype=torch.int32, device=indptr.device)
    deg = torch.empty((n,), dtype=torch.float32, device=indptr.device)
    sk = None if skip is None else skip.to(torch.uint8).contiguous()
    check(lib().gs_build_padded_adj(ptr(indptr), ptr(indices), n, max_degree, ptr(sk), seed & _U64, counter & _U64,
                                    ptr(adj), ptr(deg), stream_ptr()))
    _launched(1)
    return adj, deg


def sample_unigram(cdf, num_sampled, seed, counter, counter_dev=None):
    require_cuda(cdf, counter_dev)
    if cdf.dtype != torch.float64:
        raise TypeError("cdf must be float64")
    out = torch.empty((num_sampled,), dtype=torch.int32, device=cdf.device)
    check(lib().gs_sample_unigram(ptr(cdf), cdf.numel(), num_sampled, seed & _U64, counter & _U64, ptr(counter_dev),
                                  ptr(out), stream_ptr()))
    _launched(1 if num_sampled else 0)
    return out


def sample_unigram_unique(cdf, num_sampled, seed, counter, counter_dev=None, status=None):
    require_cuda(cdf, counter_dev, status)
    if cdf.dtype != torch.float64:
        raise TypeError("cdf must be float64")
    if status is not None and (status.dtype != torch.int32 or status.numel() < 1):
        raise TypeError("status must be an int32 tensor with >= 1 element")
    if not 0 <= int(num_sampled) <= min(_lib.MAX_UNIQUE_SAMPLED, cdf.numel()):
        raise ValueError("num_sampled must be in [0, min(%d, %d)] (got %d)" % (_lib.MAX_UNIQUE_SAMPLED, cdf.numel(), num_sampled))
    out = torch.empty((num_sampled,), dtype=torch.int32, device=cdf.device)
    ev = _probe("sample_unigram_unique")
    check(lib().gs_sample_unigram_unique(ptr(cdf), cdf.numel(), int(num_sampled), seed & _U64, counter & _U64, ptr(counter_dev),
                                         ptr(out), ptr(status), stream_ptr()))
    _launched(1 if num_sampled else 0, ev)
    return out


def sample_csr(indptr, indices, ids, k, seed, counter, replace_if_short=True, pad_id=-1, counter_dev=None):
    require_cuda(indptr, indices, ids)
    if indptr.dtype != torch.int64:
        raise TypeError("indptr must be int64")
    indices, ids = _i32(indices, "indices"), _i32(ids.reshape(-1), "ids")
    n = ids.numel()
    out = torch.empty((n, k), dtype=torch.int32, device=ids.device)
    check(lib().gs_sample_csr(ptr(indptr), ptr(indices), indptr.numel() - 1, ptr(ids), n, k, int(bool(replace_if_short)),
                              seed & _U64, counter & _U64, ptr(counter_dev), pad_id, ptr(out), stream_ptr()))
    _launched(1 if n * k else 0)
    return out


def _dtype_code(t):
    if t.dtype == torch.float32:
        return _lib.GS_F32
    if t.dtype == torch.bfloat16:
        return _lib.GS_BF16
    raise TypeError("features must be float32 or bfloat16 (got %s)" % t.dtype)


def gather_rows(feats, ids, out=None):
    if hasattr(feats, "c_table"):
        ids = _i32(ids.reshape(-1), "ids")
        n, F = ids.numel(), feats.shape[1]
        if out is None:
            out = torch.empty((n, pad_cols(F)), dtype=torch.float32, device=feats.device)[:, :F]
        check(lib().gs_gather_rows_sharded(feats.c_table(), _lib.GS_F32, F, feats.pitch, ptr(ids), n, ptr(out),
                                           out.stride(0), stream_ptr()))
        _launched(1 if n else 0)
        return out
    require_cuda(feats, ids)
    if feats.dim() != 2 or feats.stride(1) != 1:
        raise ValueError("features must be a row-major 2-D tensor")
    ids = _i32(ids.reshape(-1), "ids")
    n, F = ids.numel(), feats.shape[1]
    if out is None:
        out = torch.empty((n, F), dtype=feats.dtype, device=feats.device)
    check(lib().gs_gather_rows(ptr(feats), _dtype_code(feats), feats.shape[0], F, feats.stride(0), ptr(ids), n,
                               ptr(out), out.stride(0), stream_ptr()))
    _launched(1 if n * F else 0)
    return out


def gather_rows_f32(feats, ids=None, row0=0, n=None, out=None):
    require_cuda(feats, ids, out)
    if feats.dim() != 2 or feats.stride(1) != 1:
        raise ValueError("features must be a row-major 2-D tensor")
    F = feats.shape[1]
    if ids is not None:
        ids = _i32(ids.reshape(-1), "ids")
        n = ids.numel() if n is None else int(n)
    if n is None:
        raise ValueError("n is required without ids")
    if out is None:
        out = torch.empty((n, pad_cols(F)), dtype=torch.float32, device=feats.device)[:, :F]
    if out.dtype != torch.float32 or out.stride(1) != 1 or out.shape[0] < n:
        raise ValueError("out must be a row-major float32 matrix with >= n rows")
    check(lib().gs_gather_rows_f32(ptr(feats), _dtype_code(feats), feats.shape[0], F, feats.stride(0), ptr(ids), int(row0), n,
                                   ptr(out), out.stride(0), stream_ptr()))
    _launched(1 if n else 0)
    return out


def cast_rows_bf16(x, out=None):
    require_cuda(x, out)
    if x.dtype != torch.float32 or x.dim() != 2 or x.stride(1) != 1:
        raise ValueError("x must be a row-major float32 matrix")
    n, F = x.shape
    if out is None:
        out = torch.empty((n, pad_cols(F)), dtype=torch.bfloat16, device=x.device)[:, :F]
    if out.dtype != torch.bfloat16 or out.stride(1) != 1 or out.shape[0] < n or out.stride(0) < F:
        raise ValueError("out must be a row-major bfloat16 matrix with >= n rows")
    check(lib().gs_cast_rows_bf16(ptr(x), n, F, x.stride(0), ptr(out), out.stride(0), stream_ptr()))
    _launched(1 if n else 0)
    return out


class Seg(object):
    __slots__ = ("n", "k", "self_ids", "neigh_ids", "self_row0", "neigh_row0", "out_row0")

    def __init__(self, n, k, self_ids=None, neigh_ids=None, self_row0=0, neigh_row0=0, out_row0=0):
        self.n, self.k = int(n), int(k)
        self.self_ids = None if self_ids is None else _i32(self_ids.reshape(-1), "self_ids")
        self.neigh_ids = None if neigh_ids is None else _i32(neigh_ids.reshape(-1), "neigh_ids")
        self.self_row0, self.neigh_row0, self.out_row0 = int(self_row0), int(neigh_row0), int(out_row0)
        if self.self_ids is not None and self.self_ids.numel() < self.n:
            raise ValueError("self_ids shorter than n")
        if self.neigh_ids is not None and self.neigh_ids.numel() < self.n * self.k:
            raise ValueError("neigh_ids shorter than n*k")

    def c_struct(self):
        require_cuda(self.self_ids, self.neigh_ids)
        return Segment(ptr(self.self_ids), ptr(self.neigh_ids), self.self_row0, self.neigh_row0, self.n, self.k, 0,
                       self.out_row0)


def make_segment(n, k, self_ids=None, neigh_ids=None, self_row0=0, neigh_row0=0, out_row0=0):
    return Seg(n, k, self_ids, neigh_ids, self_row0, neigh_row0, out_row0)



def _check_out(t, rows, out_pitch, name):
    if t is None:
        return
    require_cuda(t)
    if t.dtype != torch.float32 or t.dim() != 2 or t.stride(1) != 1 or t.stride(0) != out_pitch or t.shape[0] < rows:
        raise ValueError("%s must be a float32 [>= %d, .] CUDA matrix with row stride out_pitch = %d" % (name, rows, out_pitch))


def gather_mean(src, segments, include_self=False, want_self=True, out_pitch=None, out_mean=None, out_self=None):
    if hasattr(src, "c_table"):
        return _gather_mean_sharded(src, segments, include_self, want_self, out_pitch, out_mean, out_self)
    require_cuda(src)
    if src.dtype not in (torch.float32, torch.bfloat16) or src.dim() != 2 or src.stride(1) != 1:
        raise ValueError("src must be a row-major float32 (or bfloat16) 2-D tensor")
    F = src.shape[1]
    if out_pitch is None:
        out_pitch = pad_cols(F)
    rows = max([s.out_row0 + s.n for s in segments] + [0])
    _check_out(out_mean, rows, out_pitch, "out_mean")
    _check_out(out_self if want_self else None, rows, out_pitch, "out_self")
    if out_mean is None:
        out_mean = torch.empty((rows, out_pitch), dtype=torch.float32, device=src.device)
    if want_self and out_self is None:
        out_self = torch.empty((rows, out_pitch), dtype=torch.float32, device=src.device)
    arr = (Segment * max(len(segments), 1))(*[s.c_struct() for s in segments])
    ev = _probe("gather_mean/%d" % rows)
    check(lib().gs_gather_mean(ptr(src), _dtype_code(src), src.shape[0], F, src.stride(0), arr, len(segments),
                               int(bool(include_self)), ptr(out_self) if want_self else 0, ptr(out_mean), out_pitch,
                               stream_ptr()))
    _launched(1 if rows else 0, ev)
    return (out_self if want_self else None), out_mean


def translate_ids(table, ids):
    ids = _i32(ids.reshape(-1), "ids")
    out = torch.empty_like(ids)
    check(lib().gs_translate_ids(table.c_table(), ptr(ids), ids.numel(), ptr(out), stream_ptr()))
    _launched(1 if ids.numel() else 0)
    return out


def _shard_prepare(src, segments):
    F = src.shape[1]
    locators, staging = 0, None
    by_ids = any(s.self_ids is not None or s.neigh_ids is not None for s in segments)
    if by_ids and src.world > 1 and getattr(src, "stage_halo", True):
        lists, order = {}, []
        for s in segments:
            if s.self_ids is None or s.neigh_ids is None:
                raise ValueError("with halo staging every segment of a sharded gather must address its rows by ids")
            for t in (s.self_ids, s.neigh_ids):
                key = (t.data_ptr(), t.numel())
                if key not in lists:
                    lists[key] = t
                    order.append(key)
        capacity = sum(lists[k].numel() for k in order)
        dev = src.device
        claim = torch.empty((src.shape[0],), dtype=torch.int32, device=dev)
        count = torch.empty((1,), dtype=torch.int32, device=dev)
        stage_ids = torch.empty((capacity,), dtype=torch.int32, device=dev)
        staging = torch.empty((capacity, src.pitch), dtype=torch.float32, device=dev)
        check(lib().gs_halo_begin(ptr(claim), src.shape[0], ptr(count), stream_ptr()))
        for k in order:
            check(lib().gs_halo_claim(src.c_table(), ptr(lists[k]), lists[k].numel(), ptr(claim), ptr(count), ptr(stage_ids),
                                      capacity, stream_ptr()))
        check(lib().gs_halo_fetch(src.c_table(), F, src.pitch, ptr(stage_ids), ptr(count), capacity, ptr(staging), src.pitch,
                                  stream_ptr()))
        locs = {}
        for k in order:
            locs[k] = torch.empty_like(lists[k])
            check(lib().gs_halo_translate(src.c_table(), ptr(lists[k]), lists[k].numel(), ptr(claim), ptr(locs[k]), stream_ptr()))
        _launched(2 * len(order) + 1)
        segments = [Seg(s.n, s.k, locs[(s.self_ids.data_ptr(), s.self_ids.numel())],
                        locs[(s.neigh_ids.data_ptr(), s.neigh_ids.numel())], s.self_row0, s.neigh_row0, s.out_row0)
                    for s in segments]
        locators = 2
    elif by_ids and getattr(src, "remap", None) is not None:
        done, segs = {}, []

        def tr(t):
            key = (t.data_ptr(), t.numel())
            if key not in done:
                done[key] = translate_ids(src, t)
            return done[key]

        for s in segments:
            if s.self_ids is None or s.neigh_ids is None:
                raise ValueError("with replicas every segment of a sharded gather must address its rows by ids")
            segs.append(Seg(s.n, s.k, tr(s.self_ids), tr(s.neigh_ids), s.self_row0, s.neigh_row0, s.out_row0))
        segments, locators = segs, 1
    return segments, locators, staging


def _gather_mean_sharded(src, segments, include_self, want_self, out_pitch, out_mean, out_self):
    F = src.shape[1]
    if out_pitch is None:
        out_pitch = pad_cols(F)
    rows = max([s.out_row0 + s.n for s in segments] + [0])
    _check_out(out_mean, rows, out_pitch, "out_mean")
    _check_out(out_self if want_self else None, rows, out_pitch, "out_self")
    if out_mean is None:
        out_mean = torch.empty((rows, out_pitch), dtype=torch.float32, device=src.device)
    if want_self and out_self is None:
        out_self = torch.empty((rows, out_pitch), dtype=torch.float32, device=src.device)
    segments, locators, staging = _shard_prepare(src, segments)
    arr = (Segment * max(len(segments), 1))(*[s.c_struct() for s in segments])
    ev = _probe("gather_mean/%d" % rows)
    check(lib().gs_gather_mean_sharded(src.c_table(), _lib.GS_F32, F, src.pitch, arr, len(segments),
                                       int(bool(include_self)), locators, ptr(staging), ptr(out_self) if want_self else 0,
                                       ptr(out_mean), out_pitch, stream_ptr()))
    _launched(1 if rows else 0, ev)
    return (out_self if want_self else None), out_mean


def gather_mean_images(src, segments, include_self=False, want_self=True):
    sharded = hasattr(src, "c_table")
    if not sharded:
        require_cuda(src)
        if src.dtype != torch.float32 or src.dim() != 2 or src.stride(1) != 1:
            return None
    F = src.shape[1]
    pitch = src.pitch if sharded else src.stride(0)
    if F > 1280 or pitch % 4 != 0 or (not sharded and src.data_ptr() % 16 != 0):
        return None
    rows = max([s.out_row0 + s.n for s in segments] + [0])
    if rows == 0:
        return None
    nbytes = lib().gs_gather_mean_img_bytes(rows, F, int(bool(want_self)))
    dev = src.device
    buf = torch.empty((nbytes + 1024,), dtype=torch.uint8, device=dev)
    off = (-buf.data_ptr()) % 1024
    images = buf[off:off + nbytes]
    locators, staging = 0, None
    if sharded:
        segments, locators, staging = _shard_prepare(src, segments)
    arr = (Segment * max(len(segments), 1))(*[s.c_struct() for s in segments])
    ev = _probe("gather_mean/%d" % rows)
    rc = lib().gs_gather_mean_img(0 if sharded else ptr(src), 0 if sharded else src.shape[0], src.c_table() if sharded else None,
                                  locators, ptr(staging), F, pitch, arr, len(segments), int(bool(include_self)),
                                  int(bool(want_self)), ptr(images), stream_ptr())
    if rc == -3:
        return None
    check(rc)
    _launched(1, ev)
    return images, rows


def sage_gemm_img(M, images, parts, combine=COMBINE_ADD, bias=None, act=ACT_NONE, packed=None, a_part0=0, out=None):
    _, arr, keep = _gemm_parts([(None, K, B) for (_, K, B) in parts])
    ntot = sum(p[2].shape[1] for p in parts) if (combine == COMBINE_CONCAT) else parts[0][2].shape[1]
    dev = images.device
    if out is None:
        out = torch.empty((M, ntot), dtype=torch.float32, device=dev)
    if packed is None:
        packed = PackedWeights()
    ws = packed.get(parts, arr, MATH_TF32X3, dev)
    ev = _probe("sage_gemm/%d" % M)
    check(lib().gs_sage_gemm_img(M, arr, len(parts), combine, ptr(bias), act, ptr(out), out.stride(0), ptr(ws), ptr(images),
                                 int(a_part0), stream_ptr()))
    _launched(1 if M else 0, ev)
    return out


def segment_max(x, n, k):
    require_cuda(x)
    C = x.shape[1]
    out = torch.empty((n, C), dtype=torch.float32, device=x.device)
    check(lib().gs_segment_max(ptr(x), n, k, C, x.stride(0), ptr(out), out.stride(0), stream_ptr()))
    _launched(1 if n * C else 0)
    return out


def _gemm_parts(parts):
    M = parts[0][0].shape[0] if parts[0][0] is not None else 0
    arr = (GemmPart * len(parts))()
    keep = []
    for i, (A, K, B) in enumerate(parts):
        require_cuda(A, B)
        if (A is not None and A.dtype != torch.float32) or B.dtype != torch.float32:
            raise TypeError("sage_gemm operands must be float32")
        if A is not None and (A.stride(1) != 1 or A.shape[0] != M or A.shape[1] < K):
            raise ValueError("bad A operand for part %d" % i)
        B = B.contiguous()
        if B.shape[0] != K:
            raise ValueError("part %d: B has %d rows, expected K=%d" % (i, B.shape[0], K))
        keep.append(B)
        arr[i] = GemmPart(ptr(A), A.stride(0) if A is not None else K, K, ptr(B), B.stride(0), B.shape[1])
    return M, arr, keep


class PackedWeights(object):

    def __init__(self):
        self.key, self.ws = None, None

    def get(self, parts, arr, math, dev):
        if REPACK_ALWAYS[0]:
            return self._pack(parts, arr, math, dev, None)
        key = (CACHE_EPOCH[0], math) + tuple((p[2].data_ptr(), p[2]._version, tuple(p[2].shape)) for p in parts)
        if key != self.key:
            self.ws = self._pack(parts, arr, math, dev, self.ws)
            self.key = key
        return self.ws

    @staticmethod
    def _pack(parts, arr, math, dev, ws):
        nbytes = lib().gs_sage_gemm_workspace_bytes(1, arr, len(parts), math)
        if nbytes < 0:
            check(-1)
        if ws is None or ws.numel() < nbytes:
            ws = torch.empty((max(nbytes, 1),), dtype=torch.uint8, device=dev)
        check(lib().gs_sage_gemm_pack(arr, len(parts), math, ptr(ws), stream_ptr()))
        _launched(1)
        return ws


def sage_gemm(parts, combine=COMBINE_ADD, bias=None, act=ACT_NONE, math=MATH_FP32_SIMT, out=None, packed=None):
    M, arr, keep = _gemm_parts(parts)
    ntot = sum(p[2].shape[1] for p in parts) if (combine == COMBINE_CONCAT) else parts[0][2].shape[1]
    dev = parts[0][0].device
    if out is None:
        out = torch.empty((M, ntot), dtype=torch.float32, device=dev)
    if math == MATH_FP32_SIMT or packed is None:
        ws_bytes = lib().gs_sage_gemm_workspace_bytes(M, arr, len(parts), math)
        if ws_bytes < 0:
            check(-1)
        ws = torch.empty((ws_bytes,), dtype=torch.uint8, device=dev) if ws_bytes > 0 else None
        ev = _probe("sage_gemm/%d" % M)
        check(lib().gs_sage_gemm(M, arr, len(parts), combine, ptr(bias), act, math, ptr(out), out.stride(0), ptr(ws),
                                 stream_ptr()))
        _launched((2 if ws is not None else 1) if M else 0, ev)
        return out
    ws = packed.get(parts, arr, math, dev)
    ev = _probe("sage_gemm/%d" % M)
    check(lib().gs_sage_gemm_prepacked(M, arr, len(parts), combine, ptr(bias), act, math, ptr(out), out.stride(0),
                                       ptr(ws), stream_ptr()))
    _launched(1 if M else 0, ev)
    return out


SMALL_LAYER_MAX_ROWS = 2048


def sage_layer_small(src, seg, parts, combine=COMBINE_ADD, include_self=False, bias=None, act=ACT_NONE,
                     l2_normalize=False, counter_dev=None, counter_inc=0):
    require_cuda(src, bias, counter_dev)
    if src.dtype != torch.float32 or src.stride(1) != 1:
        raise ValueError("src must be row-major float32")
    _, arr, keep = _gemm_parts([(None, K, B) for (_, K, B) in parts])
    ntot = sum(p[2].shape[1] for p in parts) if (combine == COMBINE_CONCAT) else parts[0][2].shape[1]
    rows = seg.out_row0 + seg.n
    out = torch.empty((rows, ntot), dtype=torch.float32, device=src.device)
    cseg = seg.c_struct()
    ev = _probe("sage_layer_small/%d" % rows)
    check(lib().gs_sage_layer_small(ptr(src), src.shape[0], src.shape[1], src.stride(0), cseg, int(bool(include_self)),
                                    arr, len(parts), combine, ptr(bias), act, int(bool(l2_normalize)), ptr(out),
                                    out.stride(0), ptr(counter_dev), int(counter_inc), stream_ptr()))
    _launched(1 if seg.n else 0, ev)
    return out


class PackedMlpWeights(object):

    def __init__(self):
        self.key, self.ws = None, None

    def get(self, W):
        if REPACK_ALWAYS[0]:
            return self._pack(W)
        key = (CACHE_EPOCH[0], W.data_ptr(), W._version, tuple(W.shape))
        if key != self.key:
            self.ws = self._pack(W)
            self.key = key
        return self.ws

    @staticmethod
    def _pack(W):
        K, hidden = W.shape
        nbytes = lib().gs_maxpool_mlp_workspace_bytes(K, hidden)
        ws = torch.empty((nbytes,), dtype=torch.uint8, device=W.device)
        Wc = W.contiguous()
        check(lib().gs_maxpool_mlp_pack(ptr(Wc), Wc.stride(0), K, hidden, ptr(ws), stream_ptr()))
        _launched(1)
        return ws


def maxpool_mlp_fused(table, n_groups, k, W, bias, packed, row_ids=None, row0=0, K=None, out=None, pool="max"):
    require_cuda(table, W, bias, row_ids)
    if table.dtype != torch.bfloat16 or table.stride(1) != 1:
        raise TypeError("table must be row-major bfloat16")
    K = W.shape[0] if K is None else K
    hidden = W.shape[1]
    if out is None:
        out = torch.empty((n_groups, hidden), dtype=torch.float32, device=table.device)
    ws = packed.get(W)
    if row_ids is not None:
        row_ids = _i32(row_ids.reshape(-1), "row_ids")
    ev = _probe("maxpool_mlp/%d" % n_groups)
    fn = lib().gs_meanpool_mlp_fused if pool == "mean" else lib().gs_maxpool_mlp_fused
    check(fn(ptr(table), table.shape[0], K, table.stride(0), ptr(row_ids), row0, n_groups, k,
             ptr(ws), ptr(bias), hidden, ptr(out), out.stride(0), stream_ptr()))
    _launched(1 if n_groups else 0, ev)
    return out


def dropout_site(site):
    seed, call, rate = site[:3]
    call_dev = site[3] if len(site) > 3 else None
    rate = float(rate)
    if not 0.0 <= rate < 1.0:
        raise ValueError("dropout rate must be in [0, 1) (got %r)" % (rate,))
    if call_dev is not None:
        require_cuda(call_dev)
        if call_dev.dtype != torch.int64 or call_dev.numel() < 1:
            raise TypeError("call_dev must be an int64 CUDA tensor with >= 1 element")
    return _lib.DropoutSite(int(seed) & _U64, int(call) & 0xFFFFFFFF, rate, ptr(call_dev))


def gather_mean_dropout(src, segments, neigh_sites, self_sites, include_self=False, want_self=True, out_pitch=None):
    require_cuda(src)
    if hasattr(src, "c_table") or src.dtype != torch.float32 or src.dim() != 2 or src.stride(1) != 1:
        raise ValueError("gather_mean_dropout needs a row-major float32 CUDA table")
    if len(segments) > _lib.MAX_SEGMENTS or len(neigh_sites) != len(segments) or len(self_sites) != len(segments):
        raise ValueError("gather_mean_dropout takes at most %d segments and one neighbour and one self site per segment"
                         % _lib.MAX_SEGMENTS)
    F = src.shape[1]
    if out_pitch is None:
        out_pitch = pad_cols(F)
    rows = max([s.out_row0 + s.n for s in segments] + [0])
    out_mean = torch.empty((rows, out_pitch), dtype=torch.float32, device=src.device)
    out_self = torch.empty((rows, out_pitch), dtype=torch.float32, device=src.device) if want_self else None
    nseg = max(len(segments), 1)
    arr = (Segment * nseg)(*[s.c_struct() for s in segments])
    ns = (_lib.DropoutSite * nseg)(*[dropout_site(x) for x in neigh_sites])
    ss = (_lib.DropoutSite * nseg)(*[dropout_site(x) for x in self_sites])
    ev = _probe("gather_mean_dropout/%d" % rows)
    check(lib().gs_gather_mean_dropout(ptr(src), src.shape[0], F, src.stride(0), arr, len(segments), ns, ss,
                                       int(bool(include_self)), ptr(out_self), ptr(out_mean), out_pitch, stream_ptr()))
    _launched(1 if rows else 0, ev)
    return out_self, out_mean


def dropout_apply(x, site, rows=None, group=1, scale=1.0, out=None, accumulate=False):
    require_cuda(x, out)
    group = int(group)
    if group < 1:
        raise ValueError("group must be >= 1")
    if x.dtype != torch.float32 or x.dim() != 2 or (x.stride(1) != 1 and x.shape[1] > 1):
        raise ValueError("x must be a float32 matrix with unit column stride")
    F = x.shape[1]
    rows = x.shape[0] * group if rows is None else int(rows)
    if x.shape[0] < (rows + group - 1) // group:
        raise ValueError("x has %d rows, %d needed" % (x.shape[0], (rows + group - 1) // group))
    c_site = dropout_site(site)
    if out is None:
        if accumulate:
            raise ValueError("accumulate needs out")
        out = torch.empty((rows, F), dtype=torch.float32, device=x.device)
    if out.dtype != torch.float32 or out.dim() != 2 or out.shape[0] < rows or out.shape[1] != F \
            or (out.stride(1) != 1 and F > 1):
        raise ValueError("out must be a float32 [>= %d, %d] matrix with unit column stride" % (rows, F))
    ldx, ldo = max(x.stride(0), F), max(out.stride(0), F)
    if out.data_ptr() == x.data_ptr() and (group != 1 or ldx != ldo):
        raise ValueError("in-place dropout_apply needs group == 1 and equal row strides")
    ev = _probe("dropout_apply/%d" % rows)
    check(lib().gs_dropout_apply(ptr(x), ldx, rows, F, group, float(scale), c_site, int(bool(accumulate)), ptr(out), ldo,
                                 stream_ptr()))
    _launched(1 if rows * F else 0, ev)
    return out


def _embed_lists(lists, d, who):
    if len(lists) > _lib.MAX_EMBED_LISTS:
        raise ValueError("%s takes at most %d lists" % (who, _lib.MAX_EMBED_LISTS))
    arr = (_lib.EmbedGradList * max(len(lists), 1))()
    keep = []
    dev = None
    for i, (ids, grad, group, scale) in enumerate(lists):
        require_cuda(ids, grad)
        ids = _i32(ids.reshape(-1), "ids")
        n, group = ids.numel(), int(group)
        if group < 1:
            raise ValueError("group must be >= 1")
        if grad.dtype != torch.float32 or grad.dim() != 2 or (grad.stride(1) != 1 and grad.shape[1] > 1) \
                or grad.shape[1] < d or grad.shape[0] < (n + group - 1) // group:
            raise ValueError("list %d: grad must be a float32 [>= %d, >= %d] matrix with unit column stride"
                             % (i, (n + group - 1) // group, d))
        keep.append(ids)
        dev = grad.device
        arr[i] = _lib.EmbedGradList(ptr(ids), ptr(grad), max(grad.stride(0), d), n, group, float(scale))
    return arr, keep, dev


def embedding_grad(lists, n_rows, d, out=None, sites=None):
    if sites is not None and len(sites) != len(lists):
        raise ValueError("embedding_grad: one site per list")
    arr, keep, dev = _embed_lists(lists, d, "embedding_grad")
    if out is None:
        out = torch.empty((n_rows, d), dtype=torch.float32, device=dev if dev is not None else "cuda")
    require_cuda(out)
    if out.dtype != torch.float32 or out.dim() != 2 or out.shape[0] != n_rows or out.shape[1] != d \
            or (out.stride(1) != 1 and d > 1):
        raise ValueError("out must be a float32 [%d, %d] matrix with unit column stride" % (n_rows, d))
    nbytes = lib().gs_embedding_grad_workspace_bytes(arr, len(lists), int(n_rows), int(d))
    if nbytes < 0:
        check(-1)
    ws = torch.empty((nbytes,), dtype=torch.uint8, device=out.device) if nbytes > 0 else None
    ev = _probe("embedding_grad/%d" % sum(k.numel() for k in keep))
    if sites is None:
        check(lib().gs_embedding_grad(arr, len(lists), int(n_rows), int(d), ptr(out), max(out.stride(0), d), ptr(ws), nbytes,
                                      stream_ptr()))
    else:
        c_sites = (_lib.DropoutSite * max(len(sites), 1))(*[dropout_site(s) for s in sites])
        check(lib().gs_embedding_grad_dropout(arr, c_sites, len(lists), int(n_rows), int(d), ptr(out), max(out.stride(0), d),
                                              ptr(ws), nbytes, stream_ptr()))
    _launched(3 if nbytes > 0 and n_rows * d else 0, ev)
    return out


def _fp32_table(t, name, min_cols):
    require_cuda(t)
    if t.dtype != torch.float32 or t.dim() != 2 or (t.stride(1) != 1 and t.shape[1] > 1) or t.shape[1] < min_cols:
        raise ValueError("%s must be a float32 CUDA matrix with >= %d columns and unit column stride" % (name, min_cols))


def embedding_sgd(table, lists, lr):
    _fp32_table(table, "table", 1)
    n_rows, d = table.shape
    arr, keep, _ = _embed_lists(lists, d, "embedding_sgd")
    nbytes = lib().gs_embedding_grad_workspace_bytes(arr, len(lists), int(n_rows), int(d))
    if nbytes < 0:
        check(-1)
    ws = torch.empty((nbytes,), dtype=torch.uint8, device=table.device) if nbytes > 0 else None
    ev = _probe("embedding_sgd/%d" % sum(k.numel() for k in keep))
    check(lib().gs_embedding_sgd(arr, len(lists), int(n_rows), int(d), -float(lr), ptr(table), max(table.stride(0), d), ptr(ws),
                                 nbytes, stream_ptr()))
    _launched(3 if nbytes > 0 and n_rows * d else 0, ev)
    return table


def skipgram_grad(target, context, batch1, batch2, neg):
    _fp32_table(target, "target", 1)
    d = target.shape[1]
    _fp32_table(context, "context", d + 1)
    if context.shape[0] != target.shape[0]:
        raise ValueError("target and context must have the same number of rows")
    require_cuda(batch1, batch2, neg)
    batch1, batch2, neg = _i32(batch1.reshape(-1), "batch1"), _i32(batch2.reshape(-1), "batch2"), _i32(neg.reshape(-1), "neg")
    B, S = batch1.numel(), neg.numel()
    if batch2.numel() != B or B < 1:
        raise ValueError("batch1 and batch2 must hold the same number (>= 1) of ids")
    if not 1 <= S <= _lib.MAX_UNIQUE_SAMPLED:
        raise ValueError("the number of negatives must be in [1, %d] (got %d)" % (_lib.MAX_UNIQUE_SAMPLED, S))
    dev = target.device
    f32 = dict(dtype=torch.float32, device=dev)
    wd = pad_cols(d + 1)
    out = dict(loss=torch.empty((), **f32), aff=torch.empty((B,), **f32), neg_aff=torch.empty((B, S), **f32),
               gt=torch.empty((B, pad_cols(d)), **f32)[:, :d], gc_pos=torch.empty((B, wd), **f32)[:, :d + 1],
               gc_neg=torch.empty((S, wd), **f32)[:, :d + 1])
    nbytes = lib().gs_skipgram_workspace_bytes(B, S, d)
    if nbytes < 0:
        check(-1)
    ws = torch.empty((nbytes,), dtype=torch.uint8, device=dev)
    ev = _probe("skipgram_grad/%d" % B)
    check(lib().gs_skipgram_grad(ptr(target), target.stride(0), ptr(context), context.stride(0), target.shape[0], d, ptr(batch1),
                                 ptr(batch2), B, ptr(neg), S, ptr(out["loss"]), ptr(out["aff"]), ptr(out["neg_aff"]),
                                 ptr(out["gt"]), out["gt"].stride(0), ptr(out["gc_pos"]), ptr(out["gc_neg"]), wd, ptr(ws), nbytes,
                                 stream_ptr()))
    _launched(2, ev)
    return out


def l2_normalize_rows_(x):
    require_cuda(x)
    check(lib().gs_l2_normalize_rows(ptr(x), x.shape[0], x.shape[1], x.stride(0), stream_ptr()))
    _launched(1 if x.numel() else 0)
    return x
```

include/graphsage_b200.h:

```cpp
#ifndef GRAPHSAGE_B200_H_
#define GRAPHSAGE_B200_H_

#include <stdint.h>

#ifdef __cplusplus
extern "C" {
#endif

#define GS_ABI_VERSION 2

typedef enum {
  GS_OK = 0,
  GS_ERR_INVALID_ARG = -1,
  GS_ERR_CUDA = -2,
  GS_ERR_UNSUPPORTED = -3
} gs_status;

typedef enum { GS_F32 = 0, GS_BF16 = 1 } gs_dtype;
typedef enum { GS_ACT_NONE = 0, GS_ACT_RELU = 1 } gs_act;
typedef enum {
  GS_COMBINE_ADD = 0,
  GS_COMBINE_CONCAT = 1
} gs_combine;
typedef enum {
  GS_MATH_FP32_SIMT = 0,
  GS_MATH_TF32X3 = 1,
  GS_MATH_TF32 = 2,
  GS_MATH_BF16 = 3
} gs_math;

int32_t gs_version(void);
const char* gs_last_error_string(void);
int32_t gs_set_tuning(const char* key, int32_t value);

int32_t gs_sample_padded(const int32_t* adj, int64_t n_rows, int32_t max_deg,
                         const int32_t* ids, int64_t n, int32_t k,
                         const int32_t* col_perm, uint64_t seed, uint64_t counter,
                         const uint64_t* counter_dev, int32_t* out, void* stream);

#define GS_MAX_HOPS 4
int32_t gs_sample_padded_khop(const int32_t* adj, int64_t n_rows, int32_t max_deg,
                              const int32_t* seeds, int64_t n_seeds, const int32_t* fanout_host,
                              int32_t n_hops, uint64_t seed, uint64_t counter,
                              const uint64_t* counter_dev, int32_t* const* out_host, void* stream);

int32_t gs_sample_csr(const int64_t* indptr, const int32_t* indices, int64_t n_nodes,
                      const int32_t* ids, int64_t n, int32_t k, int32_t replace_if_short,
                      uint64_t seed, uint64_t counter, const uint64_t* counter_dev,
                      int32_t pad_id, int32_t* out, void* stream);

int32_t gs_sample_unigram(const double* cdf, int64_t n, int32_t num_sampled, uint64_t seed, uint64_t counter,
                          const uint64_t* counter_dev, int32_t* out, void* stream);

#define GS_MAX_UNIQUE_SAMPLED 1024
#define GS_UNIQUE_DRAW_BUDGET (1 << 20)
int32_t gs_sample_unigram_unique(const double* cdf, int64_t n, int32_t num_sampled, uint64_t seed, uint64_t counter,
                                 const uint64_t* counter_dev, int32_t* out, int32_t* status, void* stream);

int32_t gs_build_padded_adj(const int64_t* indptr, const int32_t* indices, int64_t n_nodes, int32_t max_deg,
                            const uint8_t* skip, uint64_t seed, uint64_t counter, int32_t* adj, float* deg,
                            void* stream);

int32_t gs_perm_prefix_host(uint64_t seed, uint64_t counter, int32_t max_deg, int32_t k,
                            int32_t* out_host);

int32_t gs_gather_rows(const void* feats, int32_t dtype, int64_t n_rows, int32_t F,
                       int64_t pitch, const int32_t* ids, int64_t n, void* out,
                       int64_t out_pitch, void* stream);

#define GS_MAX_SEGMENTS 4
typedef struct {
  const int32_t* self_ids;
  const int32_t* neigh_ids;
  int64_t self_row0;
  int64_t neigh_row0;
  int64_t n;
  int32_t k;
  int32_t _pad;
  int64_t out_row0;
} gs_segment;

int32_t gs_gather_mean(const void* src, int32_t dtype, int64_t n_src_rows, int32_t F, int64_t pitch,
                       const gs_segment* segments_host, int32_t n_segments, int32_t include_self,
                       void* out_self, void* out_mean, int64_t out_pitch, void* stream);

#define GS_MAX_SHARDS 16
typedef struct {
  const void* base[GS_MAX_SHARDS];
  int64_t row_start[GS_MAX_SHARDS + 1];
  int32_t n_shards;
  int32_t my_shard;
  int64_t n_global_rows;
  int64_t zero_row;
  const int32_t* remap;
} gs_sharded_table;

int32_t gs_gather_mean_sharded(const gs_sharded_table* table_host, int32_t dtype, int32_t F, int64_t pitch,
                               const gs_segment* segments_host, int32_t n_segments, int32_t include_self,
                               int32_t ids_are_locators, const void* staging, void* out_self, void* out_mean,
                               int64_t out_pitch, void* stream);
int32_t gs_halo_begin(int32_t* claim, int64_t n_global_rows, int32_t* count, void* stream);
int32_t gs_halo_claim(const gs_sharded_table* table_host, const int32_t* ids, int64_t n, int32_t* claim, int32_t* count,
                      int32_t* stage_ids, int64_t capacity, void* stream);
int32_t gs_halo_fetch(const gs_sharded_table* table_host, int32_t F, int64_t pitch, const int32_t* stage_ids,
                      const int32_t* count, int64_t capacity, float* staging, int64_t staging_pitch, void* stream);
int32_t gs_halo_translate(const gs_sharded_table* table_host, const int32_t* ids, int64_t n, const int32_t* claim,
                          int32_t* out, void* stream);
int32_t gs_translate_ids(const gs_sharded_table* table_host, const int32_t* ids, int64_t n, int32_t* out, void* stream);
int32_t gs_gather_rows_sharded(const gs_sharded_table* table_host, int32_t dtype, int32_t F, int64_t pitch,
                               const int32_t* ids, int64_t n, void* out, int64_t out_pitch, void* stream);

int32_t gs_shard_alloc(int64_t bytes, void** dev_ptr_out);
int32_t gs_shard_free(void* dev_ptr);
int32_t gs_ipc_export(const void* dev_ptr, uint8_t* handle64_out_host);
int32_t gs_ipc_import(const uint8_t* handle64_host, void** dev_ptr_out);
int32_t gs_ipc_close(void* dev_ptr);

int32_t gs_gather_rows_f32(const void* feats, int32_t dtype, int64_t n_rows, int32_t F, int64_t pitch,
                           const int32_t* ids, int64_t row0, int64_t n, float* out, int64_t out_pitch,
                           void* stream);
int32_t gs_cast_rows_bf16(const float* x, int64_t n, int32_t F, int64_t ldx, void* out_bf16, int64_t out_pitch,
                          void* stream);

int32_t gs_rmat_degrees(int32_t scale, int64_t n_nodes, double edge_factor, double a, double b, double c, double d,
                        uint64_t seed, uint64_t mul, uint64_t mul_inv, uint64_t add, int32_t* deg_out, void* stream);
int32_t gs_rmat_fill(int32_t scale, int64_t n_nodes, double a, double b, double c, double d, uint64_t seed, uint64_t mul,
                     uint64_t mul_inv, uint64_t add, const int64_t* indptr, int32_t* indices, const int64_t* long_rows,
                     int64_t n_long, int64_t long_threshold, void* stream);

int32_t gs_segment_max(const float* x, int64_t n, int32_t k, int32_t C, int64_t ldx,
                       float* out, int64_t ldo, void* stream);

typedef struct {
  const float* A; int64_t lda; int32_t K;
  const float* B; int64_t ldb; int32_t N;
} gs_gemm_part;

int64_t gs_sage_gemm_workspace_bytes(int64_t M, const gs_gemm_part* parts_host, int32_t n_parts,
                                     int32_t math);
int32_t gs_sage_gemm(int64_t M, const gs_gemm_part* parts_host, int32_t n_parts, int32_t combine,
                     const float* bias, int32_t act, int32_t math, float* out, int64_t ldo,
                     void* workspace, void* stream);

int32_t gs_sage_gemm_pack(const gs_gemm_part* parts_host, int32_t n_parts, int32_t math, void* workspace,
                          void* stream);
int32_t gs_sage_gemm_prepacked(int64_t M, const gs_gemm_part* parts_host, int32_t n_parts, int32_t combine,
                               const float* bias, int32_t act, int32_t math, float* out, int64_t ldo,
                               const void* workspace, void* stream);

int64_t gs_gather_mean_img_bytes(int64_t rows, int32_t F, int32_t want_self);
int32_t gs_gather_mean_img(const void* src, int64_t n_src_rows, const gs_sharded_table* table_host, int32_t ids_are_locators,
                           const void* staging, int32_t F, int64_t pitch, const gs_segment* segments_host,
                           int32_t n_segments, int32_t include_self, int32_t want_self, void* images, void* stream);
int32_t gs_sage_gemm_img(int64_t M, const gs_gemm_part* parts_host, int32_t n_parts, int32_t combine, const float* bias,
                         int32_t act, float* out, int64_t ldo, const void* workspace, const void* a_images,
                         int32_t a_part0, void* stream);

int32_t gs_sage_layer_small(const float* src, int64_t n_src_rows, int32_t F, int64_t pitch,
                            const gs_segment* segment_host, int32_t include_self,
                            const gs_gemm_part* parts_host, int32_t n_parts, int32_t combine,
                            const float* bias, int32_t act, int32_t l2_normalize,
                            float* out, int64_t ldo, uint64_t* counter_dev, uint64_t counter_inc,
                            void* stream);

int64_t gs_maxpool_mlp_workspace_bytes(int32_t K, int32_t hidden);
int32_t gs_maxpool_mlp_pack(const float* Wm, int64_t ldw, int32_t K, int32_t hidden, void* workspace,
                            void* stream);
int32_t gs_maxpool_mlp_fused(const void* table_bf16, int64_t n_rows, int32_t K, int64_t pitch,
                             const int32_t* row_ids, int64_t row0, int64_t n_groups, int32_t k,
                             const void* packed_weights, const float* bias, int32_t hidden,
                             float* out, int64_t ldo, void* stream);
int32_t gs_meanpool_mlp_fused(const void* table_bf16, int64_t n_rows, int32_t K, int64_t pitch,
                              const int32_t* row_ids, int64_t row0, int64_t n_groups, int32_t k,
                              const void* packed_weights, const float* bias, int32_t hidden,
                              float* out, int64_t ldo, void* stream);

int32_t gs_pipeline_step(const void* ids_host, void* ids_dev, int64_t ids_bytes, void* const* graph_execs_host,
                         int32_t n_graphs, const void* out_dev, void* out_host, int64_t out_bytes,
                         void* h2d_stream, void* compute_stream, void* copy_stream, void* ev_ids, void* ev_done,
                         void* ev_drained);

int32_t gs_bump_counter(uint64_t* counter_dev, uint64_t inc, void* stream);

#define GS_MAX_EMBED_LISTS 8
typedef struct {
  const int32_t* ids;
  const float* grad;
  int64_t ldg;
  int64_t n;
  int32_t group;
  float scale;
} gs_embed_grad_list;

int64_t gs_embedding_grad_workspace_bytes(const gs_embed_grad_list* lists_host, int32_t n_lists, int64_t n_rows,
                                          int32_t d);
int32_t gs_embedding_grad(const gs_embed_grad_list* lists_host, int32_t n_lists, int64_t n_rows, int32_t d, float* out,
                          int64_t ldo, void* workspace, int64_t workspace_bytes, void* stream);

typedef struct {
  uint64_t seed;
  uint32_t call;
  float rate;
  const uint64_t* call_dev;
} gs_dropout_site;

int32_t gs_gather_mean_dropout(const float* src, int64_t n_src_rows, int32_t F, int64_t pitch, const gs_segment* segments_host,
                               int32_t n_segments, const gs_dropout_site* neigh_sites_host,
                               const gs_dropout_site* self_sites_host, int32_t include_self, float* out_self,
                               float* out_mean, int64_t out_pitch, void* stream);

int32_t gs_dropout_apply(const float* x, int64_t ldx, int64_t rows, int32_t F, int32_t group, float scale,
                         gs_dropout_site site, int32_t accumulate, float* out, int64_t ldo, void* stream);

int32_t gs_embedding_grad_dropout(const gs_embed_grad_list* lists_host, const gs_dropout_site* sites_host, int32_t n_lists,
                                  int64_t n_rows, int32_t d, float* out, int64_t ldo, void* workspace,
                                  int64_t workspace_bytes, void* stream);

int32_t gs_embedding_sgd(const gs_embed_grad_list* lists_host, int32_t n_lists, int64_t n_rows, int32_t d, float alpha,
                         float* table, int64_t ldt, void* workspace, int64_t workspace_bytes, void* stream);

int64_t gs_skipgram_workspace_bytes(int64_t B, int32_t S, int32_t d);
int32_t gs_skipgram_grad(const float* target, int64_t ldt, const float* context, int64_t ldc, int64_t n_rows, int32_t d,
                         const int32_t* batch1, const int32_t* batch2, int64_t B, const int32_t* neg, int32_t S, float* loss,
                         float* aff, float* neg_aff, float* gt, int64_t ldgt, float* gc_pos, float* gc_neg, int64_t ldgc,
                         void* workspace, int64_t workspace_bytes, void* stream);

int32_t gs_l2_normalize_rows(float* x, int64_t n, int32_t C, int64_t ldx, void* stream);

#ifdef __cplusplus
}
#endif
#endif
```

Measured before the change: 3.277 million.

## Reorder gather-mean output rows by self-id bucket to improve L2 locality

Adds a single-block CUB radix-sort kernel that builds a visit order for output rows, sorted by self-node id shifted into coarse buckets. The TMA bulk-copy gather kernel then walks rows in that order instead of sequentially. The aim is to improve L2 reuse when neighbouring source rows are fetched. It costs an extra kernel launch and an indirection load per row, and it only applies to batches of at most 16384 rows.

```diff
diff --git a/graphsage_b200/_lib.py b/graphsage_b200/_lib.py
--- a/graphsage_b200/_lib.py
+++ b/graphsage_b200/_lib.py
@@ -12,6 +12,7 @@
 COMBINE_ADD, COMBINE_CONCAT = 0, 1
 MATH_FP32_SIMT, MATH_TF32X3, MATH_TF32, MATH_BF16 = 0, 1, 2, 3
 MAX_SEGMENTS = 4
+GATHER_ORDER_MAX_ROWS = 16384
 
 c_i32, c_i64, c_u64, c_vp = ctypes.c_int32, ctypes.c_int64, ctypes.c_uint64, ctypes.c_void_p
 
@@ -61,8 +62,13 @@
     "gs_gather_rows": (c_i32, [c_vp, c_i32, c_i64, c_i32, c_i64, c_vp, c_i64, c_vp, c_i64, c_vp]),
     "gs_gather_mean": (c_i32, [c_vp, c_i32, c_i64, c_i32, c_i64, ctypes.POINTER(Segment), c_i32, c_i32, c_vp, c_vp,
                                c_i64, c_vp]),
+    "gs_gather_mean_ordered": (c_i32, [c_vp, c_i32, c_i64, c_i32, c_i64, ctypes.POINTER(Segment), c_i32, c_i32, c_vp, c_vp,
+                                       c_i64, c_vp, c_vp]),
+    "gs_gather_order": (c_i32, [ctypes.POINTER(Segment), c_i32, c_i64, c_vp, c_vp]),
     "gs_gather_mean_sharded": (c_i32, [ctypes.POINTER(ShardedTable), c_i32, c_i32, c_i64, ctypes.POINTER(Segment), c_i32,
                                        c_i32, c_i32, c_vp, c_vp, c_vp, c_i64, c_vp]),
+    "gs_gather_mean_sharded_ordered": (c_i32, [ctypes.POINTER(ShardedTable), c_i32, c_i32, c_i64, ctypes.POINTER(Segment),
+                                               c_i32, c_i32, c_i32, c_vp, c_vp, c_vp, c_i64, c_vp, c_vp]),
     "gs_halo_begin": (c_i32, [c_vp, c_i64, c_vp, c_vp]),
     "gs_halo_claim": (c_i32, [ctypes.POINTER(ShardedTable), c_vp, c_i64, c_vp, c_vp, c_vp, c_i64, c_vp]),
     "gs_halo_fetch": (c_i32, [ctypes.POINTER(ShardedTable), c_i32, c_i64, c_vp, c_vp, c_i64, c_vp, c_i64, c_vp]),
@@ -108,6 +114,9 @@
     "gs_embedding_grad": (c_i32, [ctypes.POINTER(EmbedGradList), c_i32, c_i64, c_i32, c_vp, c_i64, c_vp, c_i64, c_vp]),
     "gs_gather_mean_dropout": (c_i32, [c_vp, c_i64, c_i32, c_i64, ctypes.POINTER(Segment), c_i32, ctypes.POINTER(DropoutSite),
                                        ctypes.POINTER(DropoutSite), c_i32, c_vp, c_vp, c_i64, c_vp]),
+    "gs_gather_mean_dropout_ordered": (c_i32, [c_vp, c_i64, c_i32, c_i64, ctypes.POINTER(Segment), c_i32,
+                                               ctypes.POINTER(DropoutSite), ctypes.POINTER(DropoutSite), c_i32, c_vp, c_vp, c_i64,
+                                               c_vp, c_vp]),
     "gs_dropout_apply": (c_i32, [c_vp, c_i64, c_i64, c_i32, c_i32, ctypes.c_float, DropoutSite, c_i32, c_vp, c_i64, c_vp]),
     "gs_embedding_grad_dropout": (c_i32, [ctypes.POINTER(EmbedGradList), ctypes.POINTER(DropoutSite), c_i32, c_i64, c_i32, c_vp,
                                           c_i64, c_vp, c_i64, c_vp]),
@@ -139,6 +148,7 @@
             if "=" in kv:
                 k, v = kv.split("=", 1)
                 _lib.gs_set_tuning(k.strip().encode(), int(v))
+                _TUNING[k.strip()] = int(v)
     return _lib
 
 
@@ -166,8 +176,17 @@
             raise RuntimeError("graphsage_b200: tensor on %s - the hot path is CUDA-only (no CPU fallback)" % t.device)
 
 
+_TUNING = {}
+
+
 def set_tuning(key, value):
-    return lib().gs_set_tuning(key.encode(), int(value))
+    prev = lib().gs_set_tuning(key.encode(), int(value))
+    _TUNING[key] = int(value)
+    return prev
+
+
+def tuning(key, default):
+    return _TUNING.get(key, default)
 
 
 def perm_prefix_host(seed, counter, max_deg, k):
diff --git a/graphsage_b200/csrc/gather.cu b/graphsage_b200/csrc/gather.cu
--- a/graphsage_b200/csrc/gather.cu
+++ b/graphsage_b200/csrc/gather.cu
@@ -1,3 +1,9 @@
+#define CUB_WRAPPED_NAMESPACE gs_cub
+#include <cub/block/block_exchange.cuh>
+#include <cub/block/block_radix_sort.cuh>
+
+#include <algorithm>
+
 #include "common.cuh"
 
 namespace gs {
@@ -264,7 +270,8 @@
                                                                int include_self, float* __restrict__ out_self,
                                                                float* __restrict__ out_mean, int64_t out_pitch,
                                                                int row_bytes, const __grid_constant__ GatherImg img,
-                                                               const __grid_constant__ DropTab drop) {
+                                                               const __grid_constant__ DropTab drop,
+                                                               const int32_t* __restrict__ order) {
   extern __shared__ __align__(128) unsigned char smem[];
   __shared__ __align__(8) uint64_t bar[2];
   __shared__ uint32_t drop_off[2 * GS_MAX_SEGMENTS];
@@ -284,10 +291,12 @@
   const int row_f4 = row_bytes >> 4;
   const size_t buf_bytes = (size_t)kGroupRows * row_bytes;
 
-  int64_t r_issue = blockIdx.x;
+  auto row_at = [&](int64_t t) -> int64_t { return order ? (int64_t)__ldg(order + t) : t; };
+  int64_t t_issue = blockIdx.x;
+  int64_t r_issue = row_at(t_issue);
   int g_issue = 0;
   auto issue = [&](int buf) -> bool {
-    if (r_issue >= tab.total_rows) return false;
+    if (t_issue >= tab.total_rows) return false;
     int64_t i;
     const gs_segment& sg = tab.s[find_segment(tab, r_issue, i)];
     const int k = sg.k;
@@ -305,14 +314,21 @@
         bulk_g2s(smem + buf * buf_bytes + (size_t)j * row_bytes, rows_of.row(id), (uint32_t)row_bytes, &bar[buf]);
       }
     }
-    if (first + cnt >= rows_total) { r_issue += gridDim.x; g_issue = 0; } else { ++g_issue; }
+    if (first + cnt >= rows_total) {
+      t_issue += gridDim.x;
+      if (t_issue < tab.total_rows) r_issue = row_at(t_issue);
+      g_issue = 0;
+    } else {
+      ++g_issue;
+    }
     return true;
   };
 
   uint32_t phase[2] = {0u, 0u};
   int buf = 0;
   bool have = issue(0);
-  int64_t r = blockIdx.x;
+  int64_t t = blockIdx.x;
+  int64_t r = row_at(t);
   int g = 0;
   float4 acc[2];
   acc[0] = acc[1] = make_float4(0.f, 0.f, 0.f, 0.f);
@@ -374,7 +390,8 @@
           if (c < ncol4) acc[q] = make_float4(0.f, 0.f, 0.f, 0.f);
         }
       }
-      r += gridDim.x;
+      t += gridDim.x;
+      if (t < tab.total_rows) r = row_at(t);
       g = 0;
     } else {
       ++g;
@@ -829,7 +846,8 @@
 namespace gs {
 template <class Rows, bool kDrop = false>
 static int32_t launch_gather_tma2(const Rows& rows_of, int F, const SegTable& tab, int include_self, float* out_self, float* out_mean,
-                                  int64_t out_pitch, const GatherImg& img, cudaStream_t st, const DropTab* drop = nullptr) {
+                                  int64_t out_pitch, const GatherImg& img, const int32_t* order, cudaStream_t st,
+                                  const DropTab* drop = nullptr) {
   const int32_t rc_attr = ensure_dyn_smem((const void*)gather_mean_tma2_kernel<Rows, kDrop>, 200 * 1024);
   if (rc_attr != GS_OK) return rc_attr;
   const int ncol4 = (int)(out_pitch / 4);
@@ -849,8 +867,55 @@
   memset(&no_drop, 0, sizeof(no_drop));
   gather_mean_tma2_kernel<Rows, kDrop><<<(unsigned)blocks, threads, smem2, st>>>(rows_of, F, tab, include_self, out_self,
                                                                                  out_mean, out_pitch, row_bytes, img,
-                                                                                 drop ? *drop : no_drop);
+                                                                                 drop ? *drop : no_drop, order);
   return launch_check("gather_mean_tma2_kernel");
+}
+
+constexpr int kOrderThreads = 1024, kOrderMaxItems = 16;
+constexpr int kOrderRowBits = 14;
+constexpr int kOrderShift = 10;
+static_assert(kOrderThreads * kOrderMaxItems == GS_GATHER_ORDER_MAX_ROWS && (1 << kOrderRowBits) == GS_GATHER_ORDER_MAX_ROWS,
+              "gather order capacity");
+template <int kItems>
+using OrderSort = gs_cub::cub::BlockRadixSort<uint32_t, kOrderThreads, kItems>;
+template <int kItems>
+using OrderExchange = gs_cub::cub::BlockExchange<uint32_t, kOrderThreads, kItems>;
+
+template <int kItems>
+__global__ void __launch_bounds__(kOrderThreads) gather_order_kernel(const __grid_constant__ SegTable tab, int64_t n_id_space,
+                                                                     int shift, int key_bits, int32_t* __restrict__ order) {
+  extern __shared__ __align__(16) unsigned char smem[];
+  uint32_t keys[kItems];
+#pragma unroll
+  for (int q = 0; q < kItems; ++q) {
+    const int64_t r = (int64_t)q * kOrderThreads + threadIdx.x;
+    keys[q] = 0xFFFFFFFFu;
+    if (r < tab.total_rows) {
+      int64_t i;
+      const gs_segment& sg = tab.s[find_segment(tab, r, i)];
+      const int64_t id = clamp_row((int64_t)sg.self_ids[i], n_id_space);
+      keys[q] = ((uint32_t)(id >> shift) << kOrderRowBits) | (uint32_t)r;
+    }
+  }
+  OrderExchange<kItems>(*reinterpret_cast<typename OrderExchange<kItems>::TempStorage*>(smem)).StripedToBlocked(keys);
+  __syncthreads();
+  OrderSort<kItems>(*reinterpret_cast<typename OrderSort<kItems>::TempStorage*>(smem))
+      .SortBlockedToStriped(keys, kOrderRowBits, kOrderRowBits + key_bits);
+#pragma unroll
+  for (int q = 0; q < kItems; ++q) {
+    const int64_t p = (int64_t)q * kOrderThreads + threadIdx.x;
+    if (p < tab.total_rows) order[p] = (int32_t)(keys[q] & ((1u << kOrderRowBits) - 1u));
+  }
+}
+
+template <int kItems>
+static int32_t launch_gather_order(const SegTable& tab, int64_t n_id_space, int shift, int key_bits, int32_t* order,
+                                   cudaStream_t st) {
+  const int smem = (int)std::max(sizeof(typename OrderSort<kItems>::TempStorage), sizeof(typename OrderExchange<kItems>::TempStorage));
+  const int32_t rc_attr = ensure_dyn_smem((const void*)gather_order_kernel<kItems>, smem);
+  if (rc_attr != GS_OK) return rc_attr;
+  gather_order_kernel<kItems><<<1, kOrderThreads, smem, st>>>(tab, n_id_space, shift, key_bits, order);
+  return launch_check("gather_order_kernel");
 }
 }
 
@@ -896,9 +961,46 @@
   return gs::launch_check("gather_rows_simple_kernel");
 }
 
+int32_t gs_gather_order(const gs_segment* segments_host, int32_t n_segments, int64_t n_id_space, int32_t* order, void* stream) {
+  GS_REQUIRE(n_segments >= 0 && n_segments <= GS_MAX_SEGMENTS && (segments_host || n_segments == 0),
+             "gs_gather_order: bad segments");
+  GS_REQUIRE(n_id_space >= 1 && n_id_space <= 0x7fffffffLL, "gs_gather_order: n_id_space=%lld", (long long)n_id_space);
+  gs::SegTable tab;
+  memset(&tab, 0, sizeof(tab));
+  tab.n_segments = n_segments;
+  for (int s = 0; s < n_segments; ++s) {
+    tab.s[s] = segments_host[s];
+    GS_REQUIRE(tab.s[s].n >= 0, "gs_gather_order: segment %d has n=%lld", s, (long long)tab.s[s].n);
+    GS_REQUIRE(tab.s[s].n == 0 || tab.s[s].self_ids, "gs_gather_order: segment %d addresses its rows by range (no self_ids)", s);
+    tab.total_rows += tab.s[s].n;
+  }
+  GS_REQUIRE(tab.total_rows <= GS_GATHER_ORDER_MAX_ROWS, "gs_gather_order: %lld rows (max %d)", (long long)tab.total_rows,
+             GS_GATHER_ORDER_MAX_ROWS);
+  if (tab.total_rows == 0) return GS_OK;
+  GS_REQUIRE(order != nullptr, "gs_gather_order: order is NULL");
+  int id_bits = 0;
+  while (id_bits < 31 && ((n_id_space - 1) >> id_bits) != 0) ++id_bits;
+  int shift = gs::kOrderShift;
+  if (id_bits - shift > 32 - gs::kOrderRowBits) shift = id_bits - (32 - gs::kOrderRowBits);
+  int key_bits = 1;
+  while (key_bits < 32 - gs::kOrderRowBits && ((n_id_space - 1) >> (shift + key_bits)) != 0) ++key_bits;
+  const int64_t items = (tab.total_rows + gs::kOrderThreads - 1) / gs::kOrderThreads;
+  if (items <= 2) return gs::launch_gather_order<2>(tab, n_id_space, shift, key_bits, order, (cudaStream_t)stream);
+  if (items <= 4) return gs::launch_gather_order<4>(tab, n_id_space, shift, key_bits, order, (cudaStream_t)stream);
+  if (items <= 8) return gs::launch_gather_order<8>(tab, n_id_space, shift, key_bits, order, (cudaStream_t)stream);
+  return gs::launch_gather_order<16>(tab, n_id_space, shift, key_bits, order, (cudaStream_t)stream);
+}
+
 int32_t gs_gather_mean(const void* src, int32_t dtype, int64_t n_src_rows, int32_t F, int64_t pitch,
                        const gs_segment* segments_host, int32_t n_segments, int32_t include_self, void* out_self,
                        void* out_mean, int64_t out_pitch, void* stream) {
+  return gs_gather_mean_ordered(src, dtype, n_src_rows, F, pitch, segments_host, n_segments, include_self, out_self, out_mean,
+                                out_pitch, nullptr, stream);
+}
+
+int32_t gs_gather_mean_ordered(const void* src, int32_t dtype, int64_t n_src_rows, int32_t F, int64_t pitch,
+                               const gs_segment* segments_host, int32_t n_segments, int32_t include_self, void* out_self,
+                               void* out_mean, int64_t out_pitch, const int32_t* order, void* stream) {
   GS_REQUIRE(dtype == GS_F32 || dtype == GS_BF16, "gs_gather_mean: dtype %d (GS_F32 or GS_BF16)", dtype);
   GS_REQUIRE(n_segments >= 0 && n_segments <= GS_MAX_SEGMENTS, "gs_gather_mean: n_segments=%d (max %d)", n_segments,
              GS_MAX_SEGMENTS);
@@ -967,7 +1069,7 @@
     const gs::DenseRows rows_of{fsrc, n_src_rows, pitch};
     gs::GatherImg img;
     memset(&img, 0, sizeof(img));
-    return gs::launch_gather_tma2(rows_of, F, tab, include_self, (float*)out_self, (float*)out_mean, out_pitch, img, st);
+    return gs::launch_gather_tma2(rows_of, F, tab, include_self, (float*)out_self, (float*)out_mean, out_pitch, img, order, st);
   }
   if (variant >= 1 && smem <= 200 * 1024) {
     {
@@ -1065,6 +1167,15 @@
                                int32_t n_segments, const gs_dropout_site* neigh_sites_host,
                                const gs_dropout_site* self_sites_host, int32_t include_self, float* out_self,
                                float* out_mean, int64_t out_pitch, void* stream) {
+  return gs_gather_mean_dropout_ordered(src, n_src_rows, F, pitch, segments_host, n_segments, neigh_sites_host, self_sites_host,
+                                        include_self, out_self, out_mean, out_pitch, nullptr, stream);
+}
+
+int32_t gs_gather_mean_dropout_ordered(const float* src, int64_t n_src_rows, int32_t F, int64_t pitch,
+                                       const gs_segment* segments_host, int32_t n_segments,
+                                       const gs_dropout_site* neigh_sites_host, const gs_dropout_site* self_sites_host,
+                                       int32_t include_self, float* out_self, float* out_mean, int64_t out_pitch,
+                                       const int32_t* order, void* stream) {
   GS_REQUIRE(n_segments >= 0 && n_segments <= GS_MAX_SEGMENTS, "gs_gather_mean_dropout: n_segments=%d (max %d)", n_segments,
              GS_MAX_SEGMENTS);
   GS_REQUIRE((segments_host && neigh_sites_host && self_sites_host) || n_segments == 0,
@@ -1096,8 +1207,8 @@
     const gs::DenseRows rows_of{src, n_src_rows, pitch};
     gs::GatherImg img;
     memset(&img, 0, sizeof(img));
-    return gs::launch_gather_tma2<gs::DenseRows, true>(rows_of, F, tab, include_self, out_self, out_mean, out_pitch, img, st,
-                                                       &drop);
+    return gs::launch_gather_tma2<gs::DenseRows, true>(rows_of, F, tab, include_self, out_self, out_mean, out_pitch, img, order,
+                                                       st, &drop);
   }
   int64_t blocks = tab.total_rows;
   int64_t cap = (int64_t)gs::sm_count() * 8;
@@ -1221,7 +1332,7 @@
   if (src) {
     GS_REQUIRE(gs::aligned16(src) && n_src_rows > 0, "gs_gather_mean_img: table must be 16-byte aligned");
     const gs::DenseRows rows_of{(const float*)src, n_src_rows, pitch};
-    return gs::launch_gather_tma2(rows_of, F, tab, include_self, nullptr, nullptr, out_pitch, img, (cudaStream_t)stream);
+    return gs::launch_gather_tma2(rows_of, F, tab, include_self, nullptr, nullptr, out_pitch, img, nullptr, (cudaStream_t)stream);
   }
   gs::ShardRows sr;
   int32_t rc = fill_shard_tab(table_host, sr, pitch, "gs_gather_mean_img");
@@ -1230,7 +1341,7 @@
              "gs_gather_mean_img: ids_are_locators = 2 needs the staging buffer");
   sr.locators = ids_are_locators;
   sr.staging = (const float*)staging;
-  return gs::launch_gather_tma2(sr, F, tab, include_self, nullptr, nullptr, out_pitch, img, (cudaStream_t)stream);
+  return gs::launch_gather_tma2(sr, F, tab, include_self, nullptr, nullptr, out_pitch, img, nullptr, (cudaStream_t)stream);
 }
 
 int32_t gs_halo_begin(int32_t* claim, int64_t n_global_rows, int32_t* count, void* stream) {
@@ -1292,6 +1403,14 @@
                                const gs_segment* segments_host, int32_t n_segments, int32_t include_self,
                                int32_t ids_are_locators, const void* staging, void* out_self, void* out_mean,
                                int64_t out_pitch, void* stream) {
+  return gs_gather_mean_sharded_ordered(table_host, dtype, F, pitch, segments_host, n_segments, include_self, ids_are_locators,
+                                        staging, out_self, out_mean, out_pitch, nullptr, stream);
+}
+
+int32_t gs_gather_mean_sharded_ordered(const gs_sharded_table* table_host, int32_t dtype, int32_t F, int64_t pitch,
+                                       const gs_segment* segments_host, int32_t n_segments, int32_t include_self,
+                                       int32_t ids_are_locators, const void* staging, void* out_self, void* out_mean,
+                                       int64_t out_pitch, const int32_t* order, void* stream) {
   GS_REQUIRE(dtype == GS_F32, "gs_gather_mean_sharded: only GS_F32 (dtype=%d)", dtype);
   GS_REQUIRE(n_segments >= 0 && n_segments <= GS_MAX_SEGMENTS && (segments_host || n_segments == 0),
              "gs_gather_mean_sharded: bad segments");
@@ -1319,7 +1438,7 @@
   if (gs::tuning("gather_variant", 2) != 0 && ncol4 <= 2 * 160) {
     gs::GatherImg img;
     memset(&img, 0, sizeof(img));
-    return gs::launch_gather_tma2(sr, F, tab, include_self, (float*)out_self, (float*)out_mean, out_pitch, img,
+    return gs::launch_gather_tma2(sr, F, tab, include_self, (float*)out_self, (float*)out_mean, out_pitch, img, order,
                                   (cudaStream_t)stream);
   }
   int threads = ((ncol4 + 31) / 32) * 32;
diff --git a/graphsage_b200/ops.py b/graphsage_b200/ops.py
--- a/graphsage_b200/ops.py
+++ b/graphsage_b200/ops.py
@@ -233,9 +233,52 @@
         raise ValueError("%s must be a float32 [>= %d, .] CUDA matrix with row stride out_pitch = %d" % (name, rows, out_pitch))
 
 
-def gather_mean(src, segments, include_self=False, want_self=True, out_pitch=None, out_mean=None, out_self=None):
+def gather_order(segments, n_id_space):
+    total = sum(s.n for s in segments)
+    dev = next((s.self_ids.device for s in segments if s.self_ids is not None), torch.device("cuda"))
+    order = torch.empty((total,), dtype=torch.int32, device=dev)
+    arr = (Segment * max(len(segments), 1))(*[s.c_struct() for s in segments])
+    check(lib().gs_gather_order(arr, len(segments), int(n_id_space), ptr(order), stream_ptr()))
+    _launched(1 if total else 0)
+    return order
+
+
+def _bulk_copy_gather(F, pitch, out_pitch, tensors, variant_rule="dense"):
+    variant = _lib.tuning("gather_variant", 2)
+    if out_pitch // 4 > 320 or (variant_rule == "dense" and variant != 2) or (variant_rule == "sharded" and variant == 0):
+        return False
+    if variant_rule == "sharded":
+        return True
+    return (all(t.data_ptr() % 16 == 0 for t in tensors if t is not None) and pitch % 4 == 0 and out_pitch % 4 == 0
+            and (F + 3) // 4 * 4 <= pitch)
+
+
+def _visit_order(order, segments, n_id_space, bulk_copy):
+    total = sum(s.n for s in segments)
+    if isinstance(order, str):
+        if order != "auto":
+            raise ValueError("order must be 'auto', None or an int32 permutation tensor")
+        if (not bulk_copy or total == 0 or total > _lib.GATHER_ORDER_MAX_ROWS
+                or any(s.self_ids is None for s in segments if s.n)):
+            return None
+        return gather_order(segments, n_id_space)
+    if order is None:
+        return None
+    order = order.reshape(-1)
+    if order.numel() != total:
+        raise ValueError("order must hold one entry per output row (%d, got %d)" % (total, order.numel()))
+    require_cuda(order)
+    order = _i32(order, "order")
+    if not torch.cuda.is_current_stream_capturing() and not torch.equal(
+            torch.sort(order).values, torch.arange(total, dtype=torch.int32, device=order.device)):
+        raise ValueError("order must be a permutation of 0 .. %d" % (total - 1))
+    return order
+
+
+def gather_mean(src, segments, include_self=False, want_self=True, out_pitch=None, out_mean=None, out_self=None,
+                order="auto"):
     if hasattr(src, "c_table"):
-        return _gather_mean_sharded(src, segments, include_self, want_self, out_pitch, out_mean, out_self)
+        return _gather_mean_sharded(src, segments, include_self, want_self, out_pitch, out_mean, out_self, order)
     require_cuda(src)
     if src.dtype not in (torch.float32, torch.bfloat16) or src.dim() != 2 or src.stride(1) != 1:
         raise ValueError("src must be a row-major float32 (or bfloat16) 2-D tensor")
@@ -250,10 +293,12 @@
     if want_self and out_self is None:
         out_self = torch.empty((rows, out_pitch), dtype=torch.float32, device=src.device)
     arr = (Segment * max(len(segments), 1))(*[s.c_struct() for s in segments])
+    order = _visit_order(order, segments, src.shape[0], src.dtype == torch.float32 and _bulk_copy_gather(
+        F, src.stride(0), out_pitch, (src, out_mean, out_self if want_self else None)))
     ev = _probe("gather_mean/%d" % rows)
-    check(lib().gs_gather_mean(ptr(src), _dtype_code(src), src.shape[0], F, src.stride(0), arr, len(segments),
-                               int(bool(include_self)), ptr(out_self) if want_self else 0, ptr(out_mean), out_pitch,
-                               stream_ptr()))
+    check(lib().gs_gather_mean_ordered(ptr(src), _dtype_code(src), src.shape[0], F, src.stride(0), arr, len(segments),
+                                       int(bool(include_self)), ptr(out_self) if want_self else 0, ptr(out_mean), out_pitch,
+                                       ptr(order), stream_ptr()))
     _launched(1 if rows else 0, ev)
     return (out_self if want_self else None), out_mean
 
@@ -318,7 +363,7 @@
     return segments, locators, staging
 
 
-def _gather_mean_sharded(src, segments, include_self, want_self, out_pitch, out_mean, out_self):
+def _gather_mean_sharded(src, segments, include_self, want_self, out_pitch, out_mean, out_self, order):
     F = src.shape[1]
     if out_pitch is None:
         out_pitch = pad_cols(F)
@@ -329,12 +374,14 @@
         out_mean = torch.empty((rows, out_pitch), dtype=torch.float32, device=src.device)
     if want_self and out_self is None:
         out_self = torch.empty((rows, out_pitch), dtype=torch.float32, device=src.device)
+    order = _visit_order(order, segments, src.shape[0], _bulk_copy_gather(F, src.pitch, out_pitch, (), "sharded"))
     segments, locators, staging = _shard_prepare(src, segments)
     arr = (Segment * max(len(segments), 1))(*[s.c_struct() for s in segments])
     ev = _probe("gather_mean/%d" % rows)
-    check(lib().gs_gather_mean_sharded(src.c_table(), _lib.GS_F32, F, src.pitch, arr, len(segments),
-                                       int(bool(include_self)), locators, ptr(staging), ptr(out_self) if want_self else 0,
-                                       ptr(out_mean), out_pitch, stream_ptr()))
+    check(lib().gs_gather_mean_sharded_ordered(src.c_table(), _lib.GS_F32, F, src.pitch, arr, len(segments),
+                                               int(bool(include_self)), locators, ptr(staging),
+                                               ptr(out_self) if want_self else 0, ptr(out_mean), out_pitch, ptr(order),
+                                               stream_ptr()))
     _launched(1 if rows else 0, ev)
     return (out_self if want_self else None), out_mean
 
@@ -543,7 +590,8 @@
     return _lib.DropoutSite(int(seed) & _U64, int(call) & 0xFFFFFFFF, rate, ptr(call_dev))
 
 
-def gather_mean_dropout(src, segments, neigh_sites, self_sites, include_self=False, want_self=True, out_pitch=None):
+def gather_mean_dropout(src, segments, neigh_sites, self_sites, include_self=False, want_self=True, out_pitch=None,
+                        order="auto"):
     require_cuda(src)
     if hasattr(src, "c_table") or src.dtype != torch.float32 or src.dim() != 2 or src.stride(1) != 1:
         raise ValueError("gather_mean_dropout needs a row-major float32 CUDA table")
@@ -560,9 +608,12 @@
     arr = (Segment * nseg)(*[s.c_struct() for s in segments])
     ns = (_lib.DropoutSite * nseg)(*[dropout_site(x) for x in neigh_sites])
     ss = (_lib.DropoutSite * nseg)(*[dropout_site(x) for x in self_sites])
+    order = _visit_order(order, segments, src.shape[0],
+                         _bulk_copy_gather(F, src.stride(0), out_pitch, (src, out_mean, out_self), "dropout"))
     ev = _probe("gather_mean_dropout/%d" % rows)
-    check(lib().gs_gather_mean_dropout(ptr(src), src.shape[0], F, src.stride(0), arr, len(segments), ns, ss,
-                                       int(bool(include_self)), ptr(out_self), ptr(out_mean), out_pitch, stream_ptr()))
+    check(lib().gs_gather_mean_dropout_ordered(ptr(src), src.shape[0], F, src.stride(0), arr, len(segments), ns, ss,
+                                               int(bool(include_self)), ptr(out_self), ptr(out_mean), out_pitch, ptr(order),
+                                               stream_ptr()))
     _launched(1 if rows else 0, ev)
     return out_self, out_mean
 
diff --git a/include/graphsage_b200.h b/include/graphsage_b200.h
--- a/include/graphsage_b200.h
+++ b/include/graphsage_b200.h
@@ -83,6 +83,13 @@
 int32_t gs_gather_mean(const void* src, int32_t dtype, int64_t n_src_rows, int32_t F, int64_t pitch,
                        const gs_segment* segments_host, int32_t n_segments, int32_t include_self,
                        void* out_self, void* out_mean, int64_t out_pitch, void* stream);
+int32_t gs_gather_mean_ordered(const void* src, int32_t dtype, int64_t n_src_rows, int32_t F, int64_t pitch,
+                               const gs_segment* segments_host, int32_t n_segments, int32_t include_self,
+                               void* out_self, void* out_mean, int64_t out_pitch, const int32_t* order, void* stream);
+
+#define GS_GATHER_ORDER_MAX_ROWS 16384
+int32_t gs_gather_order(const gs_segment* segments_host, int32_t n_segments, int64_t n_id_space, int32_t* order,
+                        void* stream);
 
 #define GS_MAX_SHARDS 16
 typedef struct {
@@ -99,6 +106,10 @@
                                const gs_segment* segments_host, int32_t n_segments, int32_t include_self,
                                int32_t ids_are_locators, const void* staging, void* out_self, void* out_mean,
                                int64_t out_pitch, void* stream);
+int32_t gs_gather_mean_sharded_ordered(const gs_sharded_table* table_host, int32_t dtype, int32_t F, int64_t pitch,
+                                       const gs_segment* segments_host, int32_t n_segments, int32_t include_self,
+                                       int32_t ids_are_locators, const void* staging, void* out_self, void* out_mean,
+                                       int64_t out_pitch, const int32_t* order, void* stream);
 int32_t gs_halo_begin(int32_t* claim, int64_t n_global_rows, int32_t* count, void* stream);
 int32_t gs_halo_claim(const gs_sharded_table* table_host, const int32_t* ids, int64_t n, int32_t* claim, int32_t* count,
                       int32_t* stage_ids, int64_t capacity, void* stream);
@@ -208,6 +219,11 @@
                                int32_t n_segments, const gs_dropout_site* neigh_sites_host,
                                const gs_dropout_site* self_sites_host, int32_t include_self, float* out_self,
                                float* out_mean, int64_t out_pitch, void* stream);
+int32_t gs_gather_mean_dropout_ordered(const float* src, int64_t n_src_rows, int32_t F, int64_t pitch,
+                                       const gs_segment* segments_host, int32_t n_segments,
+                                       const gs_dropout_site* neigh_sites_host, const gs_dropout_site* self_sites_host,
+                                       int32_t include_self, float* out_self, float* out_mean, int64_t out_pitch,
+                                       const int32_t* order, void* stream);
 
 int32_t gs_dropout_apply(const float* x, int64_t ldx, int64_t rows, int32_t F, int32_t group, float scale,
                          gs_dropout_site site, int32_t accumulate, float* out, int64_t ldo, void* stream);
```

Result: faster. 3.439 million, median of 6 (+4.9%).
